# audiohacking/fp8-mps-metal

Hardware: AMD Instinct MI355X
Metric: FP8 _scaled_mm TFLOPS (M>=4) + GEMV HBM GB/s (M=1) vs roofline, 1/8 GPU (higher is better)
Workload: dtype fp8_e4m3fn (fp8 MFMA into fp32 accumulators); 1 GPU; gemm: M=512 K=4096 N=4096 e4m3fn, per-tensor scales, fp32 out, 20 rotating weight buffers; M=512, K=4096, N=4096, hip_graph=True, parallelism=single GPU, device=AMD Radeon Graphics, arch=gfx950:sramecc+:xnack-, compute_units=256, dev_kernarg=True

## Files before the change

### fp8-mps-metal_amd/csrc/diag/fp8mi_gemm_pc.hip

```cpp

#ifdef FP8MI_DIAG

#include "fp8mi_gemm_epi.h"

namespace {

template <int BM_, int BN_, int CWM_, int CWN_, int NL_, int NSTAGE_, int KS_, int ABL_ = 0>
struct PCfg {
    static constexpr int ABL = ABL_;
    static constexpr int BM = BM_, BN = BN_;
    static constexpr int kWavesM = CWM_, kWavesN = CWN_;
    static constexpr int kConsumers = CWM_ * CWN_;
    static constexpr int kLoaders = NL_;
    static constexpr int kWaves = kConsumers;
    static constexpr int kAllWaves = kConsumers + NL_;
    static constexpr int kThreads = kAllWaves * 64;
    static constexpr int kCThreads = kConsumers * 64;
    static constexpr int WM = BM_ / CWM_, WN = BN_ / CWN_;
    static constexpr int TM = WM / 16, TN = WN / 16;
    static constexpr int KS = KS_, NSTAGE = NSTAGE_, PF = NSTAGE_ - 1;
    static constexpr int kGroupsA = BM_ / 8, kGroupsB = BN_ / 8, kGroups = kGroupsA + kGroupsB;
    static constexpr int kStepBytes = (BM_ + BN_) * BK;
    static constexpr int kStageBytes = KS_ * kStepBytes;
    static constexpr int kRingBytes = NSTAGE_ * kStageBytes;
    static constexpr int JA = kGroupsA / NL_, JB = kGroupsB / NL_;
    static constexpr int kDma = KS_ * (JA + JB);
    static_assert(WM % 16 == 0 && WN % 16 == 0 && TM >= 1 && TN >= 1, "whole MFMA fragments per consumer");
    static_assert(kGroupsA % NL_ == 0 && kGroupsB % NL_ == 0 && NL_ % 2 == 0, "loaders stage whole groups; even count for the shared swizzle");
    static_assert(NSTAGE_ >= 3 && NSTAGE_ <= 6 && (NSTAGE_ - 1) * kDma <= 63, "vmcnt is a 6-bit counter");
    static_assert(kRingBytes + 16 <= 160 * 1024, "LDS is 160 KiB per CU");
};

typedef __attribute__((address_space(3))) uint8_t lds_u8;

template <int N>
FP8MI_DEVICE void wait_vm()
{
    asm volatile("s_waitcnt vmcnt(%0)" ::"n"(N) : "memory");
}

template <typename C>
FP8MI_DEVICE void wait_landed(int newer)
{
    constexpr int G = C::kDma;
    if (4 * G <= 63 && newer >= 4) wait_vm<(4 * G <= 63 ? 4 * G : 0)>();
    else if (3 * G <= 63 && newer == 3) wait_vm<(3 * G <= 63 ? 3 * G : 0)>();
    else if (2 * G <= 63 && newer == 2) wait_vm<(2 * G <= 63 ? 2 * G : 0)>();
    else if (newer == 1) wait_vm<G>();
    else wait_vm<0>();
}

template <typename C>
struct LoadPlan {
    uint32_t va0, vb0;
    uint32_t row0;
    uint32_t kpos;
    uint32_t sa, sb;
    int rows_a, rows_b;
    bool full;
};

template <typename C, bool TAIL>
FP8MI_DEVICE void issue_stage(const LoadPlan<C> &pl, __amdgpu_buffer_rsrc_t ra, __amdgpu_buffer_rsrc_t rb, lds_u8 *stage,
                              int lw, int k0, int64_t K)
{
#pragma unroll
    for (int q = 0; q < C::KS; ++q) {
#pragma unroll
        for (int j = 0; j < C::JA + C::JB; ++j) {
            const bool is_a = j < C::JA;
            const int jo = is_a ? j : j - C::JA;
            const int gs = q * C::kGroups + (is_a ? 0 : C::kGroupsA) + lw + jo * C::kLoaders;
            uint32_t vo = (is_a ? pl.va0 + jo * pl.sa : pl.vb0 + jo * pl.sb) + q * BK;
            if (!pl.full && (int)(pl.row0 + jo * C::kLoaders * 8) >= (is_a ? pl.rows_a : pl.rows_b)) vo = kOOB;
            if (TAIL && (int64_t)k0 + q * BK + pl.kpos >= K) vo = kOOB;
            lds_void *dst = (lds_void *)(stage + gs * 1024);
            if constexpr (C::ABL & 4) { asm volatile("" ::"v"(vo), "s"(dst)); continue; }
            if (is_a) __builtin_amdgcn_raw_ptr_buffer_load_lds(ra, dst, 16, (int)vo, k0, 0, 0);
            else __builtin_amdgcn_raw_ptr_buffer_load_lds(rb, dst, 16, (int)vo, k0, 0, 0);
        }
    }
}

template <typename C>
FP8MI_DEVICE void load_loop(const LoadPlan<C> &pl, __amdgpu_buffer_rsrc_t ra, __amdgpu_buffer_rsrc_t rb, lds_u8 *smem, int lw,
                            int s0, int ns, int64_t K)
{
    constexpr int kStageK = BK * C::KS;
    const int last = (int)((K + kStageK - 1) / kStageK) - 1;
    auto issue = [&](int s, int slot) {
        const int sg = s0 + s;
        if (sg >= last) issue_stage<C, true>(pl, ra, rb, smem + slot * C::kStageBytes, lw, sg * kStageK, K);
        else issue_stage<C, false>(pl, ra, rb, smem + slot * C::kStageBytes, lw, sg * kStageK, K);
    };
#pragma unroll
    for (int s = 0; s < C::PF; ++s)
        if (s < ns) issue(s, s);
    int fill = C::PF % C::NSTAGE;
    for (int t = 0; t < ns; ++t) {
        wait_landed<C>(min(C::PF - 1, ns - 1 - t));
        __builtin_amdgcn_s_barrier();
        if (t + C::PF < ns) issue(t + C::PF, fill);
        fill = (fill + 1 == C::NSTAGE) ? 0 : fill + 1;
    }
}

template <typename C>
FP8MI_DEVICE void read_frags(const lds_u8 *unit, int a_row0, int b_row0, uint32_t off1, uint32_t off2, i32x8 (&xf)[C::TM],
                             i32x8 (&wf)[C::TN])
{
    const lds_u8 *sa = unit + a_row0 * BK;
    const lds_u8 *sb = unit + C::kGroupsA * 1024 + b_row0 * BK;
    if constexpr (C::ABL & 1) {
        const int j = (int)(uintptr_t)unit + (int)off1;
#pragma unroll
        for (int t = 0; t < C::TN; ++t) wf[t] = i32x8{j, 1, j, 1, j, 1, j, 1};
#pragma unroll
        for (int t = 0; t < C::TM; ++t) xf[t] = i32x8{j, j, j, j, j, j, j, j};
        return;
    }
#pragma unroll
    for (int t = 0; t < C::TN; ++t) {
        i32x4 lo = *(const __attribute__((address_space(3))) i32x4 *)(sb + t * 16 * BK + off1);
        i32x4 hi = *(const __attribute__((address_space(3))) i32x4 *)(sb + t * 16 * BK + off2);
        wf[t] = i32x8{lo[0], lo[1], lo[2], lo[3], hi[0], hi[1], hi[2], hi[3]};
    }
#pragma unroll
    for (int t = 0; t < C::TM; ++t) {
        i32x4 lo = *(const __attribute__((address_space(3))) i32x4 *)(sa + t * 16 * BK + off1);
        i32x4 hi = *(const __attribute__((address_space(3))) i32x4 *)(sa + t * 16 * BK + off2);
        xf[t] = i32x8{lo[0], lo[1], lo[2], lo[3], hi[0], hi[1], hi[2], hi[3]};
    }
}

template <typename C, bool SCRUB>
FP8MI_DEVICE void mfma_unit(i32x8 (&xf)[C::TM], i32x8 (&wf)[C::TN], f32x4 (&acc)[C::TN][C::TM])
{
    if constexpr (SCRUB) {
#pragma unroll
        for (int t = 0; t < C::TM; ++t)
#pragma unroll
            for (int j = 0; j < 8; ++j) xf[t][j] = (int)scrub_nan4((uint32_t)xf[t][j]);
#pragma unroll
        for (int t = 0; t < C::TN; ++t)
#pragma unroll
            for (int j = 0; j < 8; ++j) wf[t][j] = (int)scrub_nan4((uint32_t)wf[t][j]);
    }
    if constexpr (C::ABL & 2) {
#pragma unroll
        for (int t = 0; t < C::TM; ++t) asm volatile("" ::"v"(xf[t]));
#pragma unroll
        for (int t = 0; t < C::TN; ++t) asm volatile("" ::"v"(wf[t]));
        return;
    }
#pragma unroll
    for (int tn = 0; tn < C::TN; ++tn)
#pragma unroll
        for (int tm = 0; tm < C::TM; ++tm)
            acc[tn][tm] = __builtin_amdgcn_mfma_scale_f32_16x16x128_f8f6f4(wf[tn], xf[tm], acc[tn][tm], 0, 0, 0, kScaleOne, 0, kScaleOne);
}

#define FP8MI_PC_FENCE() __builtin_amdgcn_sched_barrier(0)

template <typename C>
FP8MI_DEVICE void pin_acc(f32x4 (&acc)[C::TN][C::TM])
{
#pragma unroll
    for (int tn = 0; tn < C::TN; ++tn)
#pragma unroll
        for (int tm = 0; tm < C::TM; ++tm) asm volatile("" : "+v"(acc[tn][tm]));
}

template <typename C, bool SCRUB>
FP8MI_DEVICE void consume_loop(const lds_u8 *smem, int wm0, int wn0, uint32_t off1, uint32_t off2, int ns,
                               f32x4 (&acc)[C::TN][C::TM])
{
    static_assert(C::KS == 1 || C::KS == 2, "the pair loop below is written for one or two K-steps per stage");
#pragma unroll
    for (int tn = 0; tn < C::TN; ++tn)
#pragma unroll
        for (int tm = 0; tm < C::TM; ++tm) acc[tn][tm] = f32x4{0.0f, 0.0f, 0.0f, 0.0f};
    if (ns == 0) return;
    i32x8 xa[C::TM], wa[C::TN], xb[C::TM], wb[C::TN];
    const lds_u8 *cur = smem;
    int slot = 0;
    auto next_stage = [&]() {
        slot = (slot + 1 == C::NSTAGE) ? 0 : slot + 1;
        cur = smem + slot * C::kStageBytes;
        asm volatile("s_waitcnt lgkmcnt(0)" ::: "memory");
        __builtin_amdgcn_s_barrier();
    };
    __builtin_amdgcn_s_barrier();
    read_frags<C>(cur, wm0, wn0, off1, off2, xa, wa);
    if constexpr (C::KS == 2) {
        for (int s = 0; s < ns; ++s) {
            read_frags<C>(cur + C::kStepBytes, wm0, wn0, off1, off2, xb, wb);
            FP8MI_PC_FENCE();
            mfma_unit<C, SCRUB>(xa, wa, acc);
            pin_acc<C>(acc);
            FP8MI_PC_FENCE();
            if (s + 1 < ns) {
                next_stage();
                read_frags<C>(cur, wm0, wn0, off1, off2, xa, wa);
            }
            FP8MI_PC_FENCE();
            mfma_unit<C, SCRUB>(xb, wb, acc);
            pin_acc<C>(acc);
            FP8MI_PC_FENCE();
        }
    } else {
        int s = 0;
        for (; s + 1 < ns; s += 2) {
            next_stage();
            read_frags<C>(cur, wm0, wn0, off1, off2, xb, wb);
            FP8MI_PC_FENCE();
            mfma_unit<C, SCRUB>(xa, wa, acc);
            pin_acc<C>(acc);
            FP8MI_PC_FENCE();
            if (s + 2 < ns) {
                next_stage();
                read_frags<C>(cur, wm0, wn0, off1, off2, xa, wa);
            }
            FP8MI_PC_FENCE();
            mfma_unit<C, SCRUB>(xb, wb, acc);
            pin_acc<C>(acc);
            FP8MI_PC_FENCE();
        }
        if (s < ns) mfma_unit<C, SCRUB>(xa, wa, acc);
    }
}

template <int BM, int BN, int CWM, int CWN, int NL, int NSTAGE, int KS, int ABL>
__global__ __launch_bounds__((PCfg<BM, BN, CWM, CWN, NL, NSTAGE, KS, ABL>::kThreads)) void gemm_pc_kernel(MMParams p_in, int tiles_m, int tiles_n,
                                                                                                    int vec_store, int nwg)
{
    using C = PCfg<BM, BN, CWM, CWN, NL, NSTAGE, KS, ABL>;
    __shared__ __attribute__((aligned(16))) uint8_t smem[C::kRingBytes + kFlagBytes];
    if (threadIdx.x == 0) *(volatile int *)(smem + C::kRingBytes) = 0;
    const MMParams p = pin_params(p_in);
    FP8MI_PIN_S(tiles_m); FP8MI_PIN_S(tiles_n); FP8MI_PIN_S(vec_store); FP8MI_PIN_S(nwg);
    const EpiScalars es = load_epi_scalars(p);

    int tile_m, tile_n, kslice, wg;
    tile_of_block(blockIdx.x, nwg, tiles_m, tiles_n, tile_m, tile_n, kslice, wg);
    const int64_t m0 = (int64_t)tile_m * BM, n0 = (int64_t)tile_n * BN;

    const int lane = threadIdx.x & 63;
    const int wave = __builtin_amdgcn_readfirstlane(threadIdx.x >> 6);
    const bool is_loader = wave >= C::kConsumers;
    const int lw = wave - C::kConsumers;

    const int64_t rows_a = min((int64_t)BM, p.M - m0), rows_b = min((int64_t)BN, p.N - n0);
    constexpr int kStageK = BK * C::KS;
    const int ns_all = (int)((p.K + kStageK - 1) / kStageK);
    const int nsplit = p.split > 1 ? p.split : 1;
    const int ns_slice = (ns_all + nsplit - 1) / nsplit;
    const int s0 = kslice * ns_slice, ns = min(ns_slice, ns_all - s0);
    lds_u8 *ring = (lds_u8 *)smem;

    volatile int *flag = (volatile int *)(smem + C::kRingBytes);

    if (is_loader) {
        const int64_t bytes_a = (rows_a - 1) * p.lda + p.K, bytes_b = (rows_b - 1) * p.ldb + p.K;
        __amdgpu_buffer_rsrc_t ra = __builtin_amdgcn_make_buffer_rsrc((void *)(p.A + m0 * p.lda), 0,
                                                                       (int)min(bytes_a, (int64_t)0x7FFFFFFF), 0x00020000);
        __amdgpu_buffer_rsrc_t rb = __builtin_amdgcn_make_buffer_rsrc((void *)(p.B + n0 * p.ldb), 0,
                                                                       (int)min(bytes_b, (int64_t)0x7FFFFFFF), 0x00020000);
        LoadPlan<C> pl;
        const int row0 = lw * 8 + (lane >> 3);
        const int chunk = (lane & 7) ^ (((lw & 1) * 4 + (lane >> 4)) & 7);
        pl.row0 = (uint32_t)row0;
        pl.kpos = (uint32_t)(chunk * 16);
        pl.va0 = (uint32_t)(row0 * p.lda + chunk * 16);
        pl.vb0 = (uint32_t)(row0 * p.ldb + chunk * 16);
        pl.sa = (uint32_t)(C::kLoaders * 8 * p.lda);
        pl.sb = (uint32_t)(C::kLoaders * 8 * p.ldb);
        pl.rows_a = (int)rows_a;
        pl.rows_b = (int)rows_b;
        pl.full = rows_a == BM && rows_b == BN;
        for (int pass = 0; pass < 2; ++pass) {
            load_loop<C>(pl, ra, rb, ring, lw, s0, ns, p.K);
            __builtin_amdgcn_s_barrier();
            if (!p.nan_zero || pass == 1 || !*flag) break;
        }
        return;
    }

    const int wm0 = (wave % C::kWavesM) * C::WM, wn0 = (wave / C::kWavesM) * C::WN;
    const int fr = lane & 15, fg = lane >> 4;
    const uint32_t off1 = (uint32_t)(fr * BK + ((fg ^ (fr >> 1)) << 4));
    const uint32_t off2 = (uint32_t)(fr * BK + (((4 + fg) ^ (fr >> 1)) << 4));
    f32x4 acc[C::TN][C::TM];
    for (int pass = 0; pass < 2; ++pass) {
        if (pass == 0) consume_loop<C, false>(ring, wm0, wn0, off1, off2, ns, acc);
        else consume_loop<C, true>(ring, wm0, wn0, off1, off2, ns, acc);
        if (p.nan_zero && pass == 0 && acc_has_nan<C>(acc)) *flag = 1;
        asm volatile("s_waitcnt lgkmcnt(0)" ::: "memory");
        __builtin_amdgcn_s_barrier();
        if (!p.nan_zero || pass == 1 || !*flag) break;
    }

    if (nsplit > 1) {
        if (!splitk_combine<C>(p, acc, smem, wg, kslice, nsplit, tiles_m * tiles_n)) return;
    }

    const int rows_m = (int)rows_a, cols_n = (int)rows_b;
    if (rows_m == BM && cols_n == BN && vec_store) {
        if (p.out_dtype == FP8MI_F32) epilogue_staged<C, FP8MI_F32>(p, es, acc, smem, m0, n0, wave, wm0, wn0, lane);
        else if (p.out_dtype == FP8MI_BF16) epilogue_staged<C, FP8MI_BF16>(p, es, acc, smem, m0, n0, wave, wm0, wn0, lane);
        else epilogue_staged<C, FP8MI_F16>(p, es, acc, smem, m0, n0, wave, wm0, wn0, lane);
    } else if (p.out_dtype == FP8MI_F32) epilogue<C, FP8MI_F32>(p, es, acc, m0, n0, wm0, wn0, fr, fg, rows_m, cols_n, vec_store);
    else if (p.out_dtype == FP8MI_BF16) epilogue<C, FP8MI_BF16>(p, es, acc, m0, n0, wm0, wn0, fr, fg, rows_m, cols_n, vec_store);
    else epilogue<C, FP8MI_F16>(p, es, acc, m0, n0, wm0, wn0, fr, fg, rows_m, cols_n, vec_store);
}

template <int BM, int BN, int CWM, int CWN, int NL, int NSTAGE, int KS, int ABL = 0>
int launch_pc(const MMParams &p_in, hipStream_t s)
{
    using C = PCfg<BM, BN, CWM, CWN, NL, NSTAGE, KS, ABL>;
    MMParams p = p_in;
    const int64_t tm = (p.M + BM - 1) / BM, tn = (p.N + BN - 1) / BN;
    if (tm * tn > 0x7FFFFFFF) return FP8MI_E_UNSUPPORTED;
    const int rc = resolve_split(p, tm, tn, BM, BN, BK * KS);
    if (rc) return rc;
    const int esz = p.out_dtype == FP8MI_F32 ? 4 : 2;
    const int vec = (((p.ldc * esz) % 16) == 0 && (((uintptr_t)p.C) % 16) == 0) ? 1 : 0;
    const unsigned grid = (unsigned)(tm * tn * p.split);
    return fp8mi_launch(gemm_pc_kernel<BM, BN, CWM, CWN, NL, NSTAGE, KS, ABL>, dim3(grid), dim3(C::kThreads), s, p, (int)tm, (int)tn, vec, (int)grid);
}

}

int fp8mi_launch_gemm_pc(const MMParams &p, int variant, hipStream_t s)
{
    switch (variant) {
    case 15: return launch_pc<128, 64, 2, 2, 4, 3, 2>(p, s);
    case 16: return launch_pc<64, 128, 2, 2, 4, 3, 2>(p, s);
    case 17: return launch_pc<128, 128, 2, 2, 4, 4, 1>(p, s);
    case 20: return launch_pc<128, 64, 4, 2, 4, 3, 2>(p, s);
    case 21: return launch_pc<128, 128, 4, 2, 4, 4, 1>(p, s);
    case 22: return launch_pc<128, 64, 2, 2, 2, 3, 2>(p, s);
    case 24: return launch_pc<128, 64, 2, 2, 4, 6, 1>(p, s);
    case 25: return launch_pc<128, 64, 2, 2, 8, 3, 2>(p, s);
    case 26: return launch_pc<128, 64, 4, 2, 8, 3, 2>(p, s);
    case 27: return launch_pc<128, 128, 2, 2, 8, 4, 1>(p, s);
    case 28: return launch_pc<128, 64, 2, 2, 8, 6, 1>(p, s);
    case 208: return launch_pc<128, 64, 2, 2, 8, 3, 2, 3>(p, s);
    case 201: return launch_pc<128, 64, 2, 2, 4, 3, 2, 1>(p, s);
    case 202: return launch_pc<128, 64, 2, 2, 4, 3, 2, 2>(p, s);
    case 203: return launch_pc<128, 64, 2, 2, 4, 3, 2, 3>(p, s);
    case 204: return launch_pc<128, 64, 2, 2, 4, 3, 2, 4>(p, s);
    case 205: return launch_pc<128, 64, 2, 2, 4, 3, 2, 5>(p, s);
    case 206: return launch_pc<128, 64, 2, 2, 4, 3, 2, 6>(p, s);
    case 207: return launch_pc<128, 64, 2, 2, 4, 3, 2, 7>(p, s);
    default: return FP8MI_E_ENUM;
    }
}

#endif
```

### fp8-mps-metal_amd/csrc/fp8mi_common.h

```cpp
#pragma once

#include <hip/hip_runtime.h>
#include <hip/hip_ext.h>
#include <stdint.h>
#include <type_traits>

#include "../../include/fp8mi.h"

typedef float    f32x2  __attribute__((ext_vector_type(2)));
typedef float    f32x4  __attribute__((ext_vector_type(4)));
typedef float    f32x16 __attribute__((ext_vector_type(16)));
typedef int      i32x4  __attribute__((ext_vector_type(4)));
typedef int      i32x8  __attribute__((ext_vector_type(8)));
typedef uint32_t u32x2  __attribute__((ext_vector_type(2)));
typedef uint32_t u32x4  __attribute__((ext_vector_type(4)));
typedef _Float16 f16x2  __attribute__((ext_vector_type(2)));

#define FP8MI_DEVICE __device__ __forceinline__

struct MMParams {
    const uint8_t *A;
    const uint8_t *B;
    void *C;
    const float *scale_a;
    const float *scale_b;
    const void *bias;
    const float *scale_result;
    int64_t M, N, K;
    int64_t lda, ldb, ldc;
    int sa_row, sb_row;
    int out_dtype, bias_dtype;
    int transposed;
    int nan_zero;
    int debug;
    int split;
    uint8_t *ws;
    int64_t ws_bytes;
};

constexpr int kWsCounterBytes = 4096;

struct MxScales {
    const uint8_t *sx, *sw;
    int64_t ld_sx, ld_sw;
};

struct BwScales {
    const float *sa, *sb;
    int64_t sa_sr, sa_sk, sb_sr, sb_sk;
    int64_t nkb;
    int sh_a, sh_b;
};

struct QuantOut {
    uint8_t *out;
    int64_t ld_out;
    void *scales;
    int64_t s_sr, s_sk;
    int mx_flags;
    float *amax;
};

struct NqArgs {
    const void *in;
    int64_t rows, cols, ld_in;
    float eps;
    const void *weight, *bias, *mod_scale, *mod_shift;
    int64_t ld_mod, rows_per_mod;
    int param_dtype;
    const void *residual;
    int64_t ld_res;
    void *h_out;
    int64_t ld_h;
    QuantOut q;
    float *mean_out, *rstd_out;
};

#define FP8MI_PIN_S(x) asm volatile("" : "+s"(x))
FP8MI_DEVICE MMParams pin_params(const MMParams &p)
{
    MMParams q = p;
    FP8MI_PIN_S(q.A); FP8MI_PIN_S(q.B); FP8MI_PIN_S(q.C); FP8MI_PIN_S(q.scale_a); FP8MI_PIN_S(q.scale_b);
    FP8MI_PIN_S(q.bias); FP8MI_PIN_S(q.scale_result);
    FP8MI_PIN_S(q.M); FP8MI_PIN_S(q.N); FP8MI_PIN_S(q.K); FP8MI_PIN_S(q.lda); FP8MI_PIN_S(q.ldb); FP8MI_PIN_S(q.ldc);
    FP8MI_PIN_S(q.sa_row); FP8MI_PIN_S(q.sb_row); FP8MI_PIN_S(q.out_dtype); FP8MI_PIN_S(q.bias_dtype);
    FP8MI_PIN_S(q.transposed); FP8MI_PIN_S(q.nan_zero); FP8MI_PIN_S(q.split); FP8MI_PIN_S(q.ws); FP8MI_PIN_S(q.ws_bytes);
    return q;
}

#ifndef FP8MI_CSTORE
#define FP8MI_CSTORE 1
#endif
constexpr int kCStoreAux = FP8MI_CSTORE == 0 ? 0 : FP8MI_CSTORE == 1 ? 2 : FP8MI_CSTORE == 2 ? 17 : FP8MI_CSTORE == 3 ? 19 : FP8MI_CSTORE == 4 ? 16 : 18;
FP8MI_DEVICE void store_c16(u32x4 q, void *ptr)
{
#if FP8MI_CSTORE == 0
    *(u32x4 *)ptr = q;
#elif FP8MI_CSTORE == 1
    __builtin_nontemporal_store(q, (u32x4 *)ptr);
#elif FP8MI_CSTORE == 2
    asm volatile("global_store_dwordx4 %0, %1, off sc0 sc1" ::"v"(ptr), "v"(q) : "memory");
#elif FP8MI_CSTORE == 3
    asm volatile("global_store_dwordx4 %0, %1, off sc0 sc1 nt" ::"v"(ptr), "v"(q) : "memory");
#elif FP8MI_CSTORE == 4
    asm volatile("global_store_dwordx4 %0, %1, off sc1" ::"v"(ptr), "v"(q) : "memory");
#else
    asm volatile("global_store_dwordx4 %0, %1, off sc1 nt" ::"v"(ptr), "v"(q) : "memory");
#endif
}

FP8MI_DEVICE uint32_t scrub_nan4(uint32_t w)
{
    uint32_t n = ~(w | 0x80808080u);
    uint32_t m = ~((n + 0x7F7F7F7Fu) | 0x7F7F7F7Fu);
    m = m | (m - (m >> 7));
    return w & ~m;
}

FP8MI_DEVICE bool has_nan4(uint32_t w)
{
    uint32_t n = ~(w | 0x80808080u);
    return (~((n + 0x7F7F7F7Fu) | 0x7F7F7F7Fu)) != 0u;
}

FP8MI_DEVICE float decode_ref(uint32_t b)
{
    const uint32_t mag = b & 0x7Fu;
    if (mag == 0x7Fu) return 0.0f;
    const uint32_t sign = (b & 0x80u) << 24;
    uint32_t bits;
    if (mag >= 8u) bits = (mag << 20) + (120u << 23);
    else bits = __float_as_uint((float)mag * 0x1p-9f);
    return __uint_as_float(bits | sign);
}

FP8MI_DEVICE float decode_e5m2(uint32_t b) { return (float)__builtin_bit_cast(_Float16, (uint16_t)((b & 0xFFu) << 8)); }
FP8MI_DEVICE float decode_fmt(uint32_t b, int e5m2) { return e5m2 ? decode_e5m2(b) : __builtin_amdgcn_cvt_f32_fp8((int)b, 0); }

FP8MI_DEVICE float e2m1_value(uint32_t c)
{
    const uint32_t e = (c >> 1) & 3u, m = c & 1u;
    const float v = e == 0 ? 0.5f * (float)m : (float)((2u + m) << (e - 1)) * 0.5f;
    return (c & 8u) ? -v : v;
}

FP8MI_DEVICE float load_as_float(const void *p, int64_t i, int dtype)
{
    if (dtype == FP8MI_F32) return ((const float *)p)[i];
    if (dtype == FP8MI_F16) return (float)((const _Float16 *)p)[i];
    return (float)((const __bf16 *)p)[i];
}

FP8MI_DEVICE void store_from_float(void *p, int64_t i, float v, int dtype)
{
    if (dtype == FP8MI_F32) ((float *)p)[i] = v;
    else if (dtype == FP8MI_F16) ((_Float16 *)p)[i] = (_Float16)v;
    else ((__bf16 *)p)[i] = (__bf16)v;
}

FP8MI_DEVICE float epilogue_value(float sum, float sa, float sb, bool has_bias, float bias,
                                  bool has_sr, float sr, bool transposed = false)
{
    float r = transposed ? (sum * sb) * sa : (sum * sa) * sb;
    if (has_bias) r = r + bias;
    if (has_sr) r = r * sr;
    return r;
}

template <int CTRL>
FP8MI_DEVICE float dpp_add(float x)
{
    const int y = __builtin_amdgcn_update_dpp(0, __builtin_bit_cast(int, x), CTRL, 0xF, 0xF, false);
    return x + __builtin_bit_cast(float, y);
}

template <int P>
FP8MI_DEVICE float group_sum(float v)
{
    static_assert(P == 1 || P == 2 || P == 4 || P == 8 || P == 16, "a power of two inside a row of 16 lanes");
    if (P >= 2) v = dpp_add<0xB1>(v);
    if (P >= 4) v = dpp_add<0x4E>(v);
    if (P >= 8) v = dpp_add<0x141>(v);
    if (P >= 16) v = dpp_add<0x140>(v);
    return v;
}

FP8MI_DEVICE float wave_sum(float v)
{
    v = group_sum<16>(v);
    const int b = __builtin_bit_cast(int, v);
    const float r0 = __builtin_bit_cast(float, __builtin_amdgcn_readlane(b, 0)), r1 = __builtin_bit_cast(float, __builtin_amdgcn_readlane(b, 16)),
                r2 = __builtin_bit_cast(float, __builtin_amdgcn_readlane(b, 32)), r3 = __builtin_bit_cast(float, __builtin_amdgcn_readlane(b, 48));
    return (r0 + r1) + (r2 + r3);
}

bool fp8mi_next_profile_events(hipEvent_t *start, hipEvent_t *stop);

template <typename... KArgs>
int fp8mi_launch(void (*kernel)(KArgs...), dim3 grid, dim3 block, hipStream_t s, KArgs... args)
{
    void *argv[] = {(void *)&args...};
    hipEvent_t e0, e1;
    if (fp8mi_next_profile_events(&e0, &e1))
        return (int)hipExtLaunchKernel((const void *)kernel, grid, block, argv, 0, s, e0, e1, 0);
    return (int)hipLaunchKernel((const void *)kernel, grid, block, argv, 0, s);
}

int fp8mi_cu_count();

int fp8mi_launch_gemv(const MMParams &p, bool fp32_only, hipStream_t s, int fmt = 0);
int fp8mi_launch_gemv_variant(const MMParams &p, int id, hipStream_t s);
bool fp8mi_gemv_supported(const MMParams &p);
int fp8mi_launch_gemv_mx(const MMParams &p, hipStream_t s, int fmt = 0);
bool fp8mi_gemv_mx_supported(const MMParams &p);
int fp8mi_launch_gemv_mx_variant(const MMParams &p, int id, hipStream_t s);
int fp8mi_launch_gemm(const MMParams &p, int variant, hipStream_t s, int fmt = 0);
int fp8mi_choose_gemm_variant(const MMParams &p);
bool fp8mi_gemm_supported(const MMParams &p);
int fp8mi_launch_gemm256(const MMParams &p, int variant, hipStream_t s);
int fp8mi_launch_gemm256_fmt(const MMParams &p, int variant, hipStream_t s, int fmt);
bool fp8mi_gemm256_supported(const MMParams &p);
int fp8mi_launch_generic(const MMParams &p, hipStream_t s, int fmt = 0);
int fp8mi_launch_generic_mxfp8(const MMParams &p, const MxScales &sc, hipStream_t s);
int fp8mi_launch_gemm_mxfp8(const MMParams &p, const MxScales &sc, int variant, hipStream_t s);
bool fp8mi_gemm_mxfp8_supported(const MMParams &p, const MxScales &sc);
int fp8mi_choose_gemm_mxfp8_variant(const MMParams &p);
int fp8mi_launch_generic_mxfp4(const MMParams &p, const MxScales &sc, hipStream_t s);
int fp8mi_launch_gemm_mxfp4(const MMParams &p, const MxScales &sc, int variant, hipStream_t s);
bool fp8mi_gemm_mxfp4_supported(const MMParams &p, const MxScales &sc);
int fp8mi_launch_generic_blockwise(const MMParams &p, const BwScales &sc, hipStream_t s);
int fp8mi_launch_gemm_blockwise(const MMParams &p, const BwScales &sc, int variant, hipStream_t s);
bool fp8mi_gemm_blockwise_supported(const MMParams &p, const BwScales &sc);
int fp8mi_launch_skinny(const MMParams &p, hipStream_t s, int fmt = 0);
int fp8mi_launch_gemm_pc(const MMParams &p, int variant, hipStream_t s);
bool fp8mi_skinny_supported(const MMParams &p);
```

### fp8-mps-metal_amd/csrc/fp8mi_gemm.hip

```cpp

#include "fp8mi_gemm_epi.h"
#include "fp8mi_dispatch.h"

namespace {

template <int BM, int BN, int WM, int WN, int NSTAGE_, int MODE_ = 0, int ABL_ = 0, int KS_ = 1, int LD_ = 0, int MXS_ = 0, int FMT_ = 0>
struct Cfg {
    static constexpr int FW = (FMT_ >> 1) & 1, FX = FMT_ & 1;
    static constexpr bool OCP = FMT_ != 0;
    static_assert(FMT_ >= 0 && FMT_ <= 3 && (FMT_ == 0 || MXS_ == 0), "the block-scaled and blockwise forms are e4m3 / e2m1 only");

    static constexpr int KS = KS_;
    static constexpr int PFD = ABL_ & 7;
    static constexpr int PFA = (ABL_ >> 3) & 1;
    static constexpr int FLOOR = (ABL_ >> 4) & 3;
    static constexpr bool BREG = ((ABL_ >> 6) & 1) != 0;
    static constexpr bool XLOCAL = ((ABL_ >> 7) & 1) != 0;
    static constexpr int MODE = MODE_;
    static constexpr int NSTAGE = NSTAGE_;
    static constexpr int PF = NSTAGE_ - 1;
    static constexpr int kWavesM = BM / WM;
    static constexpr int kWavesN = BN / WN;
    static constexpr int kWaves = kWavesM * kWavesN;
    static constexpr int kThreads = kWaves * 64;
    static constexpr int kCThreads = kThreads;
    static constexpr int TM = WM / 16;
    static constexpr int TN = WN / 16;
    static constexpr int kGroupsA = BM / 8;
    static constexpr int kGroupsB = BN / 8;
    static constexpr int kGroups = kGroupsA + kGroupsB;
    static constexpr int kStepBytes = (BM + BN) * BK;
    static constexpr int kLoaders = LD_ == 0 ? kWaves : LD_;
    static constexpr int kGroupsPerWave = KS_ * kGroups / kLoaders;
    static constexpr bool MXS = MXS_ != 0;
    static constexpr bool FP4 = MXS_ == 2;
    static constexpr bool BW = MXS_ == 3;
    static constexpr int kScaleHalves = FP4 ? 2 : 1;
    static constexpr int kScalePiecesA = (BM + 63) / 64, kScalePieces = kScalePiecesA + (BN + 63) / 64;
    static constexpr int kScaleLoadsPerWave = MXS ? (KS_ * kScaleHalves * kScalePieces + kLoaders - 1) / kLoaders : 0;
    static constexpr int kScaleBytes = MXS ? (kScaleLoadsPerWave * kLoaders * 256 + 1023) / 1024 * 1024 : 0;
    static constexpr int kLoadsPerWave = kGroupsPerWave + kScaleLoadsPerWave;
    static constexpr int kStageBytes = KS_ * kStepBytes + kScaleBytes;
    static_assert(kGroupsA % kLoaders == 0 && kGroupsB % kLoaders == 0 && kLoaders % 2 == 0 && kLoaders <= kWaves,
                  "each loading wave stages whole groups of both operands; the shared swizzle needs an even count");
    static constexpr int kRingBytes = NSTAGE_ * kStageBytes;
    static_assert(NSTAGE_ >= 2 && NSTAGE_ <= 6 && (NSTAGE_ - 1) * kLoadsPerWave <= 63, "vmcnt is a 6-bit counter");
    static_assert(kRingBytes + 16 <= 160 * 1024, "LDS is 160 KiB per CU");
    static_assert(MODE_ >= 0 && MODE_ <= 2 && (MODE_ != 2 || KS_ == 1), "three orders of the loop body are built (the staggered one for KS = 1)");
};

template <typename C, bool SCRUB>
FP8MI_DEVICE void load_frags(const uint8_t *a_rows, const uint8_t *b_rows, int a_row0 , int b_row0 ,
                             uint32_t off1, uint32_t off2, i32x8 (&xf)[C::TM], i32x8 (&wf)[C::TN])
{
    const uint8_t *sa = a_rows + a_row0 * BK;
    const uint8_t *sB = b_rows + b_row0 * BK;
#pragma unroll
    for (int t = 0; t < C::TM; ++t) {
        i32x4 lo = *(const i32x4 *)(sa + t * 16 * BK + off1);
        i32x4 hi = *(const i32x4 *)(sa + t * 16 * BK + off2);
        xf[t] = i32x8{lo[0], lo[1], lo[2], lo[3], hi[0], hi[1], hi[2], hi[3]};
    }
#pragma unroll
    for (int t = 0; t < C::TN; ++t) {
        i32x4 lo = *(const i32x4 *)(sB + t * 16 * BK + off1);
        i32x4 hi = *(const i32x4 *)(sB + t * 16 * BK + off2);
        wf[t] = i32x8{lo[0], lo[1], lo[2], lo[3], hi[0], hi[1], hi[2], hi[3]};
    }
    if (SCRUB) {
#pragma unroll
        for (int t = 0; t < C::TM; ++t)
#pragma unroll
            for (int j = 0; j < 8; ++j) xf[t][j] = (int)scrub_nan4((uint32_t)xf[t][j]);
#pragma unroll
        for (int t = 0; t < C::TN; ++t)
#pragma unroll
            for (int j = 0; j < 8; ++j) wf[t][j] = (int)scrub_nan4((uint32_t)wf[t][j]);
    }
}

template <typename C>
FP8MI_DEVICE void mfma_all(const i32x8 (&xf)[C::TM], const i32x8 (&wf)[C::TN], f32x4 (&acc)[C::TN][C::TM])
{
#pragma unroll
    for (int tn = 0; tn < C::TN; ++tn)
#pragma unroll
        for (int tm = 0; tm < C::TM; ++tm)
            acc[tn][tm] = __builtin_amdgcn_mfma_scale_f32_16x16x128_f8f6f4(wf[tn], xf[tm], acc[tn][tm], C::FW, C::FX, 0,
                                                                            kScaleOne, 0, kScaleOne);
}

template <typename C, bool SCRUB>
FP8MI_DEVICE void compute_step(const uint8_t *stage, int a_row0, int b_row0, uint32_t off1, uint32_t off2,
                               f32x4 (&acc)[C::TN][C::TM])
{
    i32x8 xf[C::TM], wf[C::TN];
    load_frags<C, SCRUB>(stage, stage + C::kGroupsA * 1024, a_row0, b_row0, off1, off2, xf, wf);
    mfma_all<C>(xf, wf, acc);
}


template <typename C, bool = C::MXS> struct MxLane { };
template <typename C> struct MxLane<C, true> {
    uint32_t xo, wo;
    uint32_t rows_ok;
    int64_t kend;
};

template <typename C> struct StepScales { uint32_t x[(C::TM + 3) / 4], w[(C::TN + 3) / 4]; };

template <typename C>
FP8MI_DEVICE void load_scales(const uint8_t *sc, const MxLane<C, true> &ml, int64_t kstep, StepScales<C> &s, int koff = 0)
{
    const bool kin = kstep * BK + koff < ml.kend;
#pragma unroll
    for (int t = 0; t < (C::TM + 3) / 4; ++t) s.x[t] = 0u;
#pragma unroll
    for (int t = 0; t < (C::TN + 3) / 4; ++t) s.w[t] = 0u;
#pragma unroll
    for (int t = 0; t < C::TM; ++t) {
        const uint32_t b = sc[ml.xo + t * 64];
        s.x[t >> 2] |= ((kin && ((ml.rows_ok >> t) & 1u)) ? b : 0x7Fu) << (8 * (t & 3));
    }
#pragma unroll
    for (int t = 0; t < C::TN; ++t) {
        const uint32_t b = sc[ml.wo + t * 64];
        s.w[t >> 2] |= ((kin && ((ml.rows_ok >> (16 + t)) & 1u)) ? b : 0x7Fu) << (8 * (t & 3));
    }
}

FP8MI_DEVICE f32x4 mfma_mx(i32x8 w, i32x8 x, f32x4 c, uint32_t sw, int ow, uint32_t sx, int ox)
{
#define FP8MI_MX_CASE(a, b) \
    case a * 4 + b: return __builtin_amdgcn_mfma_scale_f32_16x16x128_f8f6f4(w, x, c, 0, 0, a, (int)sw, b, (int)sx);
    switch (ow * 4 + ox) {
        FP8MI_MX_CASE(0, 0) FP8MI_MX_CASE(0, 1) FP8MI_MX_CASE(0, 2) FP8MI_MX_CASE(0, 3)
        FP8MI_MX_CASE(1, 0) FP8MI_MX_CASE(1, 1) FP8MI_MX_CASE(1, 2) FP8MI_MX_CASE(1, 3)
        FP8MI_MX_CASE(2, 0) FP8MI_MX_CASE(2, 1) FP8MI_MX_CASE(2, 2) FP8MI_MX_CASE(2, 3)
        FP8MI_MX_CASE(3, 0) FP8MI_MX_CASE(3, 1) FP8MI_MX_CASE(3, 2) FP8MI_MX_CASE(3, 3)
    default: return c;
    }
#undef FP8MI_MX_CASE
}

template <typename C>
FP8MI_DEVICE void mfma_all(const i32x8 (&xf)[C::TM], const i32x8 (&wf)[C::TN], f32x4 (&acc)[C::TN][C::TM], const StepScales<C> &s)
{
#pragma unroll
    for (int tn = 0; tn < C::TN; ++tn)
#pragma unroll
        for (int tm = 0; tm < C::TM; ++tm)
            acc[tn][tm] = mfma_mx(wf[tn], xf[tm], acc[tn][tm], s.w[tn >> 2], tn & 3, s.x[tm >> 2], tm & 3);
}


FP8MI_DEVICE f32x4 mfma_mx4(i32x8 w, i32x8 x, f32x4 c, uint32_t sw, int ow, uint32_t sx, int ox)
{
#define FP8MI_MX4_CASE(a, b) \
    case a * 4 + b: return __builtin_amdgcn_mfma_scale_f32_16x16x128_f8f6f4(w, x, c, 4, 4, a, (int)sw, b, (int)sx);
    switch (ow * 4 + ox) {
        FP8MI_MX4_CASE(0, 0) FP8MI_MX4_CASE(0, 1) FP8MI_MX4_CASE(0, 2) FP8MI_MX4_CASE(0, 3)
        FP8MI_MX4_CASE(1, 0) FP8MI_MX4_CASE(1, 1) FP8MI_MX4_CASE(1, 2) FP8MI_MX4_CASE(1, 3)
        FP8MI_MX4_CASE(2, 0) FP8MI_MX4_CASE(2, 1) FP8MI_MX4_CASE(2, 2) FP8MI_MX4_CASE(2, 3)
        FP8MI_MX4_CASE(3, 0) FP8MI_MX4_CASE(3, 1) FP8MI_MX4_CASE(3, 2) FP8MI_MX4_CASE(3, 3)
    default: return c;
    }
#undef FP8MI_MX4_CASE
}

FP8MI_DEVICE i32x8 frag_hi(i32x8 f) { return __builtin_shufflevector(f, f, 4, 5, 6, 7, 4, 5, 6, 7); }

template <typename C>
FP8MI_DEVICE void mfma_step_fp4(const i32x8 (&xf)[C::TM], const i32x8 (&wf)[C::TN], f32x4 (&acc)[C::TN][C::TM], const uint8_t *sc,
                                const MxLane<C> &ml, int64_t kstep)
{
    StepScales<C> s0, s1;
    load_scales<C>(sc, ml, kstep, s0);
    load_scales<C>(sc + C::kScalePieces * 256, ml, kstep, s1, 64);
#pragma unroll
    for (int tn = 0; tn < C::TN; ++tn)
#pragma unroll
        for (int tm = 0; tm < C::TM; ++tm)
            acc[tn][tm] = mfma_mx4(wf[tn], xf[tm], acc[tn][tm], s0.w[tn >> 2], tn & 3, s0.x[tm >> 2], tm & 3);
#pragma unroll
    for (int tn = 0; tn < C::TN; ++tn)
#pragma unroll
        for (int tm = 0; tm < C::TM; ++tm)
            acc[tn][tm] = mfma_mx4(frag_hi(wf[tn]), frag_hi(xf[tm]), acc[tn][tm], s1.w[tn >> 2], tn & 3, s1.x[tm >> 2], tm & 3);
}

template <typename C>
FP8MI_DEVICE void fold_bw(f32x4 &acc, const f32x4 &pb, float sa, const f32x4 &sb)
{
#pragma unroll
    for (int j = 0; j < 4; ++j) {
        float s = sa * sb[j];
        asm("" : "+v"(s));
        float r = __builtin_fmaf(pb[j], s, acc[j]);
        asm("" : "+v"(r));
        acc[j] = r;
    }
}

template <typename C>
FP8MI_DEVICE void mfma_fold_bw(const i32x8 (&xf)[C::TM], const i32x8 (&wf)[C::TN], f32x4 (&acc)[C::TN][C::TM], const uint8_t *sc,
                               const MxLane<C> &ml)
{
    float sa[C::TM];
    f32x4 sb[C::TN];
#pragma unroll
    for (int t = 0; t < C::TM; ++t) sa[t] = *(const float *)(sc + ml.xo + t * 64);
#pragma unroll
    for (int t = 0; t < C::TN; ++t) sb[t] = *(const f32x4 *)(sc + ml.wo + t * 64);
    f32x4 prev = f32x4{0.0f, 0.0f, 0.0f, 0.0f};
#pragma unroll
    for (int i = 0; i < C::TN * C::TM; ++i) {
        const int tn = i / C::TM, tm = i % C::TM;
        const f32x4 cur = __builtin_amdgcn_mfma_scale_f32_16x16x128_f8f6f4(wf[tn], xf[tm], f32x4{0.0f, 0.0f, 0.0f, 0.0f}, 0, 0, 0,
                                                                          kScaleOne, 0, kScaleOne);
        if (i > 0) fold_bw<C>(acc[(i - 1) / C::TM][(i - 1) % C::TM], prev, sa[(i - 1) % C::TM], sb[(i - 1) / C::TM]);
        prev = cur;
    }
    constexpr int kLast = C::TN * C::TM - 1;
    fold_bw<C>(acc[kLast / C::TM][kLast % C::TM], prev, sa[kLast % C::TM], sb[kLast / C::TM]);
}

template <typename C, bool SCRUB>
FP8MI_DEVICE void compute_step(const uint8_t *stage, int q, int a_row0, int b_row0, uint32_t off1, uint32_t off2,
                               const MxLane<C> &ml, int64_t kstep, f32x4 (&acc)[C::TN][C::TM])
{
    if constexpr (C::BW) {
        i32x8 xf[C::TM], wf[C::TN];
        const uint8_t *st = stage + q * C::kStepBytes;
        load_frags<C, SCRUB>(st, st + C::kGroupsA * 1024, a_row0, b_row0, off1, off2, xf, wf);
        mfma_fold_bw<C>(xf, wf, acc, stage + C::KS * C::kStepBytes + q * C::kScalePieces * 256, ml);
    } else if constexpr (C::FP4) {
        i32x8 xf[C::TM], wf[C::TN];
        const uint8_t *st = stage + q * C::kStepBytes;
        load_frags<C, false>(st, st + C::kGroupsA * 1024, a_row0, b_row0, off1, off2, xf, wf);
        mfma_step_fp4<C>(xf, wf, acc, stage + C::KS * C::kStepBytes + q * 2 * C::kScalePieces * 256, ml, kstep);
    } else if constexpr (C::MXS) {
        i32x8 xf[C::TM], wf[C::TN];
        StepScales<C> sc;
        const uint8_t *st = stage + q * C::kStepBytes;
        load_frags<C, SCRUB>(st, st + C::kGroupsA * 1024, a_row0, b_row0, off1, off2, xf, wf);
        load_scales<C>(stage + C::KS * C::kStepBytes + q * C::kScalePieces * 256, ml, kstep, sc);
        mfma_all<C>(xf, wf, acc, sc);
    } else {
        compute_step<C, SCRUB>(stage + q * C::kStepBytes, a_row0, b_row0, off1, off2, acc);
    }
}

template <typename C, bool = C::MXS> struct ScaleStage { };
template <typename C> struct ScaleStage<C, true> {
    __amdgpu_buffer_rsrc_t rx, rw;
    uint32_t voff[C::kScaleLoadsPerWave];
    bool is_x[C::kScaleLoadsPerWave];
    uint32_t kx, kw;
    int nkb;
    int q[C::kScaleLoadsPerWave];
};

template <typename C>
struct StagePlan {
    uint32_t va0, vb0;
    uint32_t row0;
    uint32_t kpos;
    uint32_t sa, sb;
    int rows_a, rows_b;
    bool full;
    uint32_t pf_off;
    u32x4 pf_rsrc;
    int pf_waves;
    mutable u32x4 bsink;
    ScaleStage<C> sc;
};

template <typename C, bool TAIL>
FP8MI_DEVICE void issue_stage(const StagePlan<C> &pl, __amdgpu_buffer_rsrc_t ra, __amdgpu_buffer_rsrc_t rb,
                              uint8_t *stage, int wave, int k0, int64_t K)
{
    constexpr int JA = C::kGroupsA / C::kLoaders, JB = C::kGroupsB / C::kLoaders, JS = JA + JB;
    if (C::kLoaders < C::kWaves && wave >= C::kLoaders) return;
#pragma unroll
    for (int j = 0; j < C::kGroupsPerWave; ++j) {
        const int q = j / JS, jj = j % JS;
        const bool is_a = jj < JA;
        const int jo = is_a ? jj : jj - JA;
        const int gs = q * C::kGroups + (is_a ? 0 : C::kGroupsA) + wave + jo * C::kLoaders;
        uint32_t vo = (is_a ? pl.va0 + jo * pl.sa : pl.vb0 + jo * pl.sb) + q * BK;
        if (!pl.full && (int)(pl.row0 + jo * C::kLoaders * 8) >= (is_a ? pl.rows_a : pl.rows_b)) vo = kOOB;
        if (TAIL && (int64_t)k0 + q * BK + pl.kpos >= K) vo = kOOB;
        lds_void *dst = (lds_void *)(stage + gs * 1024);
        if (is_a) __builtin_amdgcn_raw_ptr_buffer_load_lds(ra, dst, 16, (int)vo, k0, 0, 0);
        else if constexpr (C::BREG) asm volatile("buffer_load_dwordx4 %0, %1, %2, %3 offen" : "+v"(pl.bsink) : "v"(vo), "s"(pl.pf_rsrc), "s"((uint32_t)k0) : "memory");
        else __builtin_amdgcn_raw_ptr_buffer_load_lds(rb, dst, 16, (int)vo, k0, 0, 0);
    }
    if constexpr (C::BW) {
        const int kb = k0 / BK;
#pragma unroll
        for (int j = 0; j < C::kScaleLoadsPerWave; ++j) {
            lds_void *dst = (lds_void *)(stage + C::KS * C::kStepBytes + (wave + j * C::kLoaders) * 256);
            const uint32_t vo = kb + pl.sc.q[j] < pl.sc.nkb ? pl.sc.voff[j] + (uint32_t)kb * (pl.sc.is_x[j] ? pl.sc.kx : pl.sc.kw) : kOOB;
            __builtin_amdgcn_raw_ptr_buffer_load_lds(pl.sc.is_x[j] ? pl.sc.rx : pl.sc.rw, dst, 4, (int)vo, 0, 0, 0);
        }
    } else if constexpr (C::MXS) {
#pragma unroll
        for (int j = 0; j < C::kScaleLoadsPerWave; ++j) {
            lds_void *dst = (lds_void *)(stage + C::KS * C::kStepBytes + (wave + j * C::kLoaders) * 256);
            __builtin_amdgcn_raw_ptr_buffer_load_lds(pl.sc.is_x[j] ? pl.sc.rx : pl.sc.rw, dst, 4, (int)pl.sc.voff[j], C::FP4 ? k0 / 16 : k0 / 32, 0, 0);
        }
    }
}

#ifdef FP8MI_STAMP
#define STAMP(var)                                                                 \
    do {                                                                           \
        __builtin_amdgcn_sched_barrier(0);                                         \
        unsigned long long t_;                                                     \
        asm volatile("s_memtime %0\n\ts_waitcnt lgkmcnt(0)" : "=s"(t_)::"memory"); \
        __builtin_amdgcn_sched_barrier(0);                                         \
        var = t_;                                                                  \
    } while (0)
__device__ unsigned long long g_stamp[256 * 32];
#else
#define STAMP(var) do { } while (0)
#endif

template <int N>
FP8MI_DEVICE void wait_loads_and_lds()
{
    asm volatile("s_waitcnt vmcnt(%0) lgkmcnt(0)" ::"n"(N) : "memory");
}

template <typename C>
FP8MI_DEVICE void wait_stage(int newer_stages)
{
    constexpr int G = C::kLoadsPerWave;
    if (5 * G <= 63 && newer_stages >= 5) wait_loads_and_lds<(5 * G <= 63 ? 5 * G : 0)>();
    else if (4 * G <= 63 && newer_stages == 4) wait_loads_and_lds<(4 * G <= 63 ? 4 * G : 0)>();
    else if (3 * G <= 63 && newer_stages == 3) wait_loads_and_lds<(3 * G <= 63 ? 3 * G : 0)>();
    else if (2 * G <= 63 && newer_stages == 2) wait_loads_and_lds<(2 * G <= 63 ? 2 * G : 0)>();
    else if (newer_stages == 1) wait_loads_and_lds<G>();
    else wait_loads_and_lds<0>();
}

template <typename C>
FP8MI_DEVICE void issue_any(const StagePlan<C> &pl, __amdgpu_buffer_rsrc_t ra, __amdgpu_buffer_rsrc_t rb,
                            uint8_t *stage, int wave, int step, int nk, bool ktail, int64_t K)
{
    if (ktail && step == nk - 1) issue_stage<C, true>(pl, ra, rb, stage, wave, step * (BK * C::KS), K);
    else issue_stage<C, false>(pl, ra, rb, stage, wave, step * (BK * C::KS), K);
}

FP8MI_DEVICE void prefetch_stage(uint32_t &sink, uint32_t voff, u32x4 rsrc, uint32_t koff)
{
    asm volatile("buffer_load_dword %0, %1, %2, %3 offen" : "+v"(sink) : "v"(voff), "s"(rsrc), "s"(koff) : "memory");
}

template <typename C, bool SCRUB>
FP8MI_DEVICE void run_tile(const MMParams &p, uint8_t *smem, const StagePlan<C> &pl, __amdgpu_buffer_rsrc_t ra,
                           __amdgpu_buffer_rsrc_t rb, int wave, int wm0, int wn0, uint32_t off1, uint32_t off2,
                           int ks0, int nk, int rot, const MxLane<C> &ml, f32x4 (&acc)[C::TN][C::TM])
{
#pragma unroll
    for (int tn = 0; tn < C::TN; ++tn)
#pragma unroll
        for (int tm = 0; tm < C::TM; ++tm) acc[tn][tm] = f32x4{0.0f, 0.0f, 0.0f, 0.0f};

    const int64_t K = p.K;
    const int nk_all = (int)((K + BK * C::KS - 1) / (BK * C::KS));
    const bool ktail = (K % (BK * C::KS)) != 0;
    if (nk == 0) return;
    unsigned long long p0_ = 0, p1_ = 0, p2_ = 0; (void)p0_; (void)p1_; (void)p2_;
    STAMP(p0_);

    int ks = rot;
    auto next_ks = [&]() { const int r = ks; ks = (ks + 1 == nk) ? 0 : ks + 1; return ks0 + r; };
    uint32_t sink = 0;
    auto prefetch = [&](int stage) {
        if (C::PFD > 0 && wave < pl.pf_waves + C::PFA) prefetch_stage(sink, pl.pf_off, pl.pf_rsrc, (uint32_t)((ks0 + min(stage, nk - 1)) * (BK * C::KS)));
    };

#pragma unroll
    for (int s = 0; s < C::PF; ++s)
        if (s < nk) issue_any<C>(pl, ra, rb, smem + s * C::kStageBytes, wave, next_ks(), nk_all, ktail, K);
#pragma unroll
    for (int s = 0; s < C::PFD; ++s) prefetch(C::PF + s);

    STAMP(p1_);
    int slot = 0;
    int fill = C::PF % C::NSTAGE;
    unsigned long long c_wait = 0, c_bar = 0, c_issue = 0, c_comp = 0, s0 = 0, s1 = 0, s2 = 0, s3 = 0, s4 = 0;
    (void)c_wait; (void)c_bar; (void)c_issue; (void)c_comp; (void)s0; (void)s1; (void)s2; (void)s3; (void)s4;
    for (int t = 0; t < nk; ++t) {
        const int64_t kst = (int64_t)(ks0 + (rot + t < nk ? rot + t : rot + t - nk)) * C::KS;
        STAMP(s0);
        wait_stage<C>(min(C::PF - 1, nk - 1 - t));
        STAMP(s1);
        __builtin_amdgcn_s_barrier();
        STAMP(s2);
        if constexpr (C::MODE == 1) {
            i32x8 xf[C::TM], wf[C::TN];
            const uint8_t *st = smem + slot * C::kStageBytes;
            if constexpr (C::FLOOR == 0) load_frags<C, SCRUB>(st, st + C::kGroupsA * 1024, wm0, wn0, off1, off2, xf, wf);
            __builtin_amdgcn_sched_barrier(0);
            if (t + C::PF < nk) {
                issue_any<C>(pl, ra, rb, smem + fill * C::kStageBytes, wave, next_ks(), nk_all, ktail, K);
                prefetch(t + C::PF + C::PFD);
            }
            STAMP(s3);
            if constexpr (C::FLOOR == 0 && C::BW) {
                mfma_fold_bw<C>(xf, wf, acc, st + C::KS * C::kStepBytes, ml);
#pragma unroll
                for (int q = 1; q < C::KS; ++q) compute_step<C, SCRUB>(st, q, wm0, wn0, off1, off2, ml, kst + q, acc);
            } else if constexpr (C::FLOOR == 0 && C::FP4) {
                mfma_step_fp4<C>(xf, wf, acc, st + C::KS * C::kStepBytes, ml, kst);
#pragma unroll
                for (int q = 1; q < C::KS; ++q) compute_step<C, SCRUB>(st, q, wm0, wn0, off1, off2, ml, kst + q, acc);
            } else if constexpr (C::FLOOR == 0 && C::MXS) {
                StepScales<C> sc;
                load_scales<C>(st + C::KS * C::kStepBytes, ml, kst, sc);
                mfma_all<C>(xf, wf, acc, sc);
#pragma unroll
                for (int q = 1; q < C::KS; ++q) compute_step<C, SCRUB>(st, q, wm0, wn0, off1, off2, ml, kst + q, acc);
            } else if constexpr (C::FLOOR == 0) {
                mfma_all<C>(xf, wf, acc);
#pragma unroll
                for (int q = 1; q < C::KS; ++q)
                    compute_step<C, SCRUB>(st + q * C::kStepBytes, wm0, wn0, off1, off2, acc);
            }
        } else {
            if (t + C::PF < nk) {
                issue_any<C>(pl, ra, rb, smem + fill * C::kStageBytes, wave, next_ks(), nk_all, ktail, K);
                prefetch(t + C::PF + C::PFD);
            }
            STAMP(s3);
            if constexpr (C::FLOOR == 0 && C::MXS) {
#pragma unroll
                for (int q = 0; q < C::KS; ++q) compute_step<C, SCRUB>(smem + slot * C::kStageBytes, q, wm0, wn0, off1, off2, ml, kst + q, acc);
            } else if constexpr (C::FLOOR == 0) {
#pragma unroll
                for (int q = 0; q < C::KS; ++q)
                    compute_step<C, SCRUB>(smem + slot * C::kStageBytes + q * C::kStepBytes, wm0, wn0, off1, off2, acc);
            }
        }
        STAMP(s4);
        c_wait += s1 - s0; c_bar += s2 - s1; c_issue += s3 - s2; c_comp += s4 - s3;
#ifdef FP8MI_STAMP
        if (t == 5 && (threadIdx.x & 63) == 0 && blockIdx.x < 256 && (wave == 0 || wave == C::kWaves / 2)) {
            unsigned long long *o = g_stamp + blockIdx.x * 32 + 16 + (wave ? 5 : 0);
            o[0] = s0; o[1] = s1; o[2] = s2; o[3] = s3; o[4] = s4;
        }
#endif
        slot = (slot + 1 == C::NSTAGE) ? 0 : slot + 1;
        fill = (fill + 1 == C::NSTAGE) ? 0 : fill + 1;
    }
#ifdef FP8MI_STAMP
    if ((threadIdx.x & 63) == 0 && blockIdx.x < 256 && (wave == 0 || wave == C::kWaves / 2)) {
        unsigned long long *o = g_stamp + blockIdx.x * 32 + (wave ? 8 : 0);
        o[0] = c_wait; o[1] = c_bar; o[2] = c_issue; o[3] = c_comp; o[4] = nk;
    }
#endif
    if (C::PFD > 0) asm volatile("" ::"v"(sink));
#ifdef FP8MI_STAMP
    STAMP(p2_);
    if ((threadIdx.x & 63) == 0 && blockIdx.x < 256 && wave == 0) {
        unsigned long long *o = g_stamp + blockIdx.x * 32 + 26;
        o[0] = p0_; o[1] = p1_; o[2] = p2_;
    }
#endif
}

template <typename C, bool SCRUB>
FP8MI_DEVICE void run_tile_staggered(const MMParams &p, uint8_t *smem, const StagePlan<C> &pl, __amdgpu_buffer_rsrc_t ra,
                                     __amdgpu_buffer_rsrc_t rb, int wave, int wm0, int wn0, uint32_t off1, uint32_t off2,
                                     int ks0, int nk, int rot, const MxLane<C> &ml, f32x4 (&acc)[C::TN][C::TM])
{
    static_assert(C::KS == 1, "one K-step per ring stage");
    static_assert(!C::FP4 && !C::BW, "the MXFP4 and blockwise instances are built on the MODE 0 / 1 loops");
#pragma unroll
    for (int tn = 0; tn < C::TN; ++tn)
#pragma unroll
        for (int tm = 0; tm < C::TM; ++tm) acc[tn][tm] = f32x4{0.0f, 0.0f, 0.0f, 0.0f};
    const int64_t K = p.K;
    const int nk_all = (int)((K + BK - 1) / BK);
    const bool ktail = (K % BK) != 0;
    if (nk == 0) return;
    int ks = rot;
    auto next_ks = [&]() { const int r = ks; ks = (ks + 1 == nk) ? 0 : ks + 1; return ks0 + r; };
#pragma unroll
    for (int s = 0; s < C::PF; ++s)
        if (s < nk) issue_any<C>(pl, ra, rb, smem + s * C::kStageBytes, wave, next_ks(), nk_all, ktail, K);
    int slot = 0, fill = C::PF % C::NSTAGE;
    auto advance = [&]() {
        slot = (slot + 1 == C::NSTAGE) ? 0 : slot + 1;
        fill = (fill + 1 == C::NSTAGE) ? 0 : fill + 1;
    };
    i32x8 xf[C::TM], wf[C::TN];
    StepScales<C> sc;
#define FP8MI_READ_STEP(st, t)                                                                                                   \
    do {                                                                                                                         \
        load_frags<C, SCRUB>(st, st + C::kGroupsA * 1024, wm0, wn0, off1, off2, xf, wf);                                          \
        if constexpr (C::MXS) load_scales<C>(st + C::kStepBytes, ml, (int64_t)(ks0 + (rot + t < nk ? rot + t : rot + t - nk)), sc); \
    } while (0)
#define FP8MI_MULTIPLY()                                        \
    do {                                                        \
        if constexpr (C::MXS) mfma_all<C>(xf, wf, acc, sc);     \
        else mfma_all<C>(xf, wf, acc);                          \
    } while (0)
    if (wave < C::kWaves / 2) {
        for (int t = 0; t < nk; ++t) {
            wait_stage<C>(min(C::PF - 1, nk - 1 - t));
            __builtin_amdgcn_s_barrier();
            const uint8_t *st = smem + slot * C::kStageBytes;
            FP8MI_READ_STEP(st, t);
            __builtin_amdgcn_sched_barrier(0);
            if (t + C::PF < nk) issue_any<C>(pl, ra, rb, smem + fill * C::kStageBytes, wave, next_ks(), nk_all, ktail, K);
            FP8MI_MULTIPLY();
            advance();
        }
    } else {
        for (int t = 0; t < nk; ++t) {
            wait_stage<C>(min(C::PF - 1, nk - 1 - t));
            __builtin_amdgcn_s_barrier();
            if (t > 0) {
                FP8MI_MULTIPLY();
#pragma unroll
                for (int tn = 0; tn < C::TN; ++tn)
#pragma unroll
                    for (int tm = 0; tm < C::TM; ++tm) asm volatile("" : "+v"(acc[tn][tm]));
            }
            asm volatile("" ::: "memory");
            __builtin_amdgcn_sched_barrier(0);
            if (t + C::PF < nk) issue_any<C>(pl, ra, rb, smem + fill * C::kStageBytes, wave, next_ks(), nk_all, ktail, K);
            const uint8_t *st = smem + slot * C::kStageBytes;
            FP8MI_READ_STEP(st, t);
            advance();
        }
        FP8MI_MULTIPLY();
    }
#undef FP8MI_READ_STEP
#undef FP8MI_MULTIPLY
}

template <typename C, bool SCRUB>
FP8MI_DEVICE void run_tile_any(const MMParams &p, uint8_t *smem, const StagePlan<C> &pl, __amdgpu_buffer_rsrc_t ra,
                               __amdgpu_buffer_rsrc_t rb, int wave, int wm0, int wn0, uint32_t off1, uint32_t off2,
                               int ks0, int nk, int rot, const MxLane<C> &ml, f32x4 (&acc)[C::TN][C::TM])
{
    if constexpr (C::MODE == 2) run_tile_staggered<C, SCRUB>(p, smem, pl, ra, rb, wave, wm0, wn0, off1, off2, ks0, nk, rot, ml, acc);
    else run_tile<C, SCRUB>(p, smem, pl, ra, rb, wave, wm0, wn0, off1, off2, ks0, nk, rot, ml, acc);
}

using MxArgs = MxScales;
struct MxParams {
    MMParams mm;
    MxArgs s;
};

template <typename C, typename S>
FP8MI_DEVICE void gemm_tile(const MMParams &p, const S &mx, const EpiScalars &es, uint8_t *smem, int tiles_m, int tiles_n,
                            int vec_store, int nwg)
{
    constexpr int BM = C::kWavesM * (C::TM * 16), BN = C::kWavesN * (C::TN * 16), WM = C::TM * 16, WN = C::TN * 16;
    if (!C::FP4 && !C::OCP && threadIdx.x == 0) *(volatile int *)(smem + C::kRingBytes) = 0;

    unsigned long long k0_ = 0, k1_ = 0, k2_ = 0; (void)k0_; (void)k1_; (void)k2_;
    STAMP(k0_);
#ifdef FP8MI_STAMP
    const unsigned long long r0_ = __builtin_amdgcn_s_memrealtime();
#endif
    int tile_m, tile_n, kslice, wg;
    tile_of_block(blockIdx.x, nwg, tiles_m, tiles_n, tile_m, tile_n, kslice, wg);
    if constexpr (C::XLOCAL) {
        const int q = nwg >> 3, r = nwg & 7, xcd = blockIdx.x & 7;
        const int wg_all = (xcd < r ? xcd * (q + 1) : r * (q + 1) + (xcd - r) * q) + ((int)blockIdx.x >> 3);
        const int split = max(p.split, 1);
        wg = wg_all / split;
        kslice = wg_all - wg * split;
        tile_m = wg % tiles_m;
        tile_n = wg / tiles_m;
    }
    const int n_tiles = tiles_m * tiles_n;
    const int64_t m0 = (int64_t)tile_m * BM, n0 = (int64_t)tile_n * BN;

    const int lane = threadIdx.x & 63;
    const int wave = __builtin_amdgcn_readfirstlane(threadIdx.x >> 6);
    const int wm0 = (wave % C::kWavesM) * WM;
    const int wn0 = (wave / C::kWavesM) * WN;

    const int64_t rows_a = min((int64_t)BM, p.M - m0), rows_b = min((int64_t)BN, p.N - n0);
    const int64_t bytes_a = (rows_a - 1) * p.lda + p.K, bytes_b = (rows_b - 1) * p.ldb + p.K;
    __amdgpu_buffer_rsrc_t ra = __builtin_amdgcn_make_buffer_rsrc((void *)(p.A + m0 * p.lda), 0,
                                                                   (int)min(bytes_a, (int64_t)0x7FFFFFFF), 0x00020000);
    __amdgpu_buffer_rsrc_t rb = __builtin_amdgcn_make_buffer_rsrc((void *)(p.B + n0 * p.ldb), 0,
                                                                   (int)min(bytes_b, (int64_t)0x7FFFFFFF), 0x00020000);

    StagePlan<C> pl;
    {
        const int row0 = wave * 8 + (lane >> 3);
        const int chunk = (lane & 7) ^ (((wave & 1) * 4 + (lane >> 4)) & 7);
        pl.row0 = (uint32_t)row0;
        pl.kpos = (uint32_t)(chunk * 16);
        pl.va0 = (uint32_t)(row0 * p.lda + chunk * 16);
        pl.vb0 = (uint32_t)(row0 * p.ldb + chunk * 16);
        pl.sa = (uint32_t)(C::kLoaders * 8 * p.lda);
        pl.sb = (uint32_t)(C::kLoaders * 8 * p.ldb);
        pl.rows_a = (int)rows_a;
        pl.rows_b = (int)rows_b;
        pl.full = rows_a == BM && rows_b == BN;
        pl.pf_off = kOOB;
        pl.pf_waves = 0;
        pl.bsink = u32x4{0u, 0u, 0u, 0u};
        if constexpr (C::BREG) {
            static_assert(C::PFD == 0, "BREG borrows the prefetch descriptor");
            const uint64_t pbr = (uint64_t)(p.B + n0 * p.ldb);
            pl.pf_rsrc = u32x4{(uint32_t)__builtin_amdgcn_readfirstlane((int)(uint32_t)pbr),
                               (uint32_t)__builtin_amdgcn_readfirstlane((int)((uint32_t)(pbr >> 32) & 0xFFFFu)),
                               (uint32_t)__builtin_amdgcn_readfirstlane((int)min(bytes_b, (int64_t)0x7FFFFFFF)), 0x00020000u};
            for (int o = (int)threadIdx.x * 16; o < C::kRingBytes; o += C::kThreads * 16) *(u32x4 *)(smem + o) = u32x4{0u, 0u, 0u, 0u};
            __syncthreads();
        }
        if (C::PFD > 0) {
            constexpr int kLines = BN * C::KS / 4;
            static_assert(C::PFD == 0 || kLines <= 64, "one prefetch instruction per stage");
            const int gm = min(4, tiles_m - (tile_m & ~3)), nshare = gm >= 4 ? 4 : (gm >= 2 ? 2 : 1);
            pl.pf_waves = nshare == 1 ? 0 : 4 / nshare;
            const int quarter = (tile_m % nshare) * (4 / nshare) + wave;
            const int li = (quarter & 3) * kLines + lane, prow = li / C::KS, pk = li % C::KS;
            if (lane < kLines && prow < (int)rows_b && (p.K % (BK * C::KS)) == 0) pl.pf_off = (uint32_t)(prow * p.ldb + pk * BK);
            const uint64_t pb = (uint64_t)(p.B + n0 * p.ldb);
            pl.pf_rsrc = u32x4{(uint32_t)__builtin_amdgcn_readfirstlane((int)(uint32_t)pb),
                               (uint32_t)__builtin_amdgcn_readfirstlane((int)((uint32_t)(pb >> 32) & 0xFFFFu)),
                               (uint32_t)__builtin_amdgcn_readfirstlane((int)min(bytes_b, (int64_t)0x7FFFFFFF)), 0x00020000u};
            if (C::PFA && wave == pl.pf_waves) {
                constexpr int kLinesA = BM * C::KS / 8;
                static_assert(!C::PFA || kLinesA <= 64, "one prefetch instruction per stage");
                const int lia = (tile_n & 7) * kLinesA + lane, arow = lia / C::KS, ak = lia % C::KS;
                pl.pf_off = (lane < kLinesA && arow < (int)rows_a && (p.K % (BK * C::KS)) == 0) ? (uint32_t)(arow * p.lda + ak * BK) : kOOB;
                const uint64_t pa = (uint64_t)(p.A + m0 * p.lda);
                pl.pf_rsrc = u32x4{(uint32_t)__builtin_amdgcn_readfirstlane((int)(uint32_t)pa),
                                   (uint32_t)__builtin_amdgcn_readfirstlane((int)((uint32_t)(pa >> 32) & 0xFFFFu)),
                                   (uint32_t)__builtin_amdgcn_readfirstlane((int)min(bytes_a, (int64_t)0x7FFFFFFF)), 0x00020000u};
            }
        }
    }

    const int fr = lane & 15, fg = lane >> 4;
    const uint32_t off1 = (uint32_t)(fr * BK + ((fg ^ (fr >> 1)) << 4));
    const uint32_t off2 = (uint32_t)(fr * BK + (((4 + fg) ^ (fr >> 1)) << 4));

    MxLane<C> ml;
    if constexpr (C::BW) {
        const int64_t bx0 = m0 >> mx.sh_a, bw0 = n0 >> mx.sh_b;
        const int64_t nbx = ((m0 + rows_a - 1) >> mx.sh_a) - bx0 + 1, nbw = ((n0 + rows_b - 1) >> mx.sh_b) - bw0 + 1;
        const int64_t ext_x = ((nbx - 1) * mx.sa_sr + (mx.nkb - 1) * mx.sa_sk + 1) * 4, ext_w = ((nbw - 1) * mx.sb_sr + (mx.nkb - 1) * mx.sb_sk + 1) * 4;
        pl.sc.rx = __builtin_amdgcn_make_buffer_rsrc((void *)(mx.sa + bx0 * mx.sa_sr), 0, (int)min(ext_x, (int64_t)0x7FFFFFFF), 0x00020000);
        pl.sc.rw = __builtin_amdgcn_make_buffer_rsrc((void *)(mx.sb + bw0 * mx.sb_sr), 0, (int)min(ext_w, (int64_t)0x7FFFFFFF), 0x00020000);
        pl.sc.kx = (uint32_t)(mx.sa_sk * 4);
        pl.sc.kw = (uint32_t)(mx.sb_sk * 4);
        pl.sc.nkb = (int)mx.nkb;
#pragma unroll
        for (int j = 0; j < C::kScaleLoadsPerWave; ++j) {
            const int idx = wave + j * C::kLoaders, q = idx / C::kScalePieces, part = idx - q * C::kScalePieces;
            const bool is_x = part < C::kScalePiecesA;
            const int row = (is_x ? part : part - C::kScalePiecesA) * 64 + lane;
            const bool ok = idx < C::KS * C::kScalePieces && row < (is_x ? rows_a : rows_b);
            const int64_t rb = is_x ? ((m0 + row) >> mx.sh_a) - bx0 : ((n0 + row) >> mx.sh_b) - bw0;
            pl.sc.voff[j] = ok ? (uint32_t)(rb * (is_x ? mx.sa_sr : mx.sb_sr) * 4 + q * (is_x ? pl.sc.kx : pl.sc.kw)) : kOOB;
            pl.sc.is_x[j] = is_x;
            pl.sc.q[j] = q;
        }
        ml.xo = (uint32_t)((wm0 + fr) * 4);
        ml.wo = (uint32_t)(C::kScalePiecesA * 256 + (wn0 + fg * 4) * 4);
        ml.rows_ok = 0;
        ml.kend = 0;
    } else if constexpr (C::MXS) {
        pl.sc.rx = __builtin_amdgcn_make_buffer_rsrc((void *)(mx.sx + m0 * mx.ld_sx), 0, (int)min(rows_a * mx.ld_sx, (int64_t)0x7FFFFFFF), 0x00020000);
        pl.sc.rw = __builtin_amdgcn_make_buffer_rsrc((void *)(mx.sw + n0 * mx.ld_sw), 0, (int)min(rows_b * mx.ld_sw, (int64_t)0x7FFFFFFF), 0x00020000);
#pragma unroll
        for (int j = 0; j < C::kScaleLoadsPerWave; ++j) {
            const int idx = wave + j * C::kLoaders, q = idx / C::kScalePieces, part = idx - q * C::kScalePieces;
            const bool is_x = part < C::kScalePiecesA;
            const int row = (is_x ? part : part - C::kScalePiecesA) * 64 + lane;
            const bool ok = idx < C::KS * C::kScaleHalves * C::kScalePieces && row < (is_x ? rows_a : rows_b);
            pl.sc.voff[j] = ok ? (uint32_t)(row * (is_x ? mx.ld_sx : mx.ld_sw) + q * 4) : kOOB;
            pl.sc.is_x[j] = is_x;
        }
        ml.xo = (uint32_t)((wm0 + fr) * 4 + fg);
        ml.wo = (uint32_t)(C::kScalePiecesA * 256 + (wn0 + fr) * 4 + fg);
        uint32_t ok = 0;
#pragma unroll
        for (int t = 0; t < C::TM; ++t) ok |= (wm0 + t * 16 + fr < rows_a) ? 1u << t : 0u;
#pragma unroll
        for (int t = 0; t < C::TN; ++t) ok |= (wn0 + t * 16 + fr < rows_b) ? 1u << (16 + t) : 0u;
        ml.rows_ok = ok;
        ml.kend = p.K - (C::FP4 ? 16 : 32) * fg;
    }

    const int nk_all = (int)((p.K + BK * C::KS - 1) / (BK * C::KS));
    const int nsplit = p.split > 1 ? p.split : 1;
    const int nk_slice = (nk_all + nsplit - 1) / nsplit;
    const int ks0 = kslice * nk_slice, nk = min(nk_slice, nk_all - ks0);
    const int rot = 0;

    f32x4 acc[C::TN][C::TM];
    if constexpr (C::FLOOR == 2) {
#pragma unroll
        for (int tn = 0; tn < C::TN; ++tn)
#pragma unroll
            for (int tm = 0; tm < C::TM; ++tm) acc[tn][tm] = f32x4{0.0f, 0.0f, 0.0f, 0.0f};
    } else
    run_tile_any<C, false>(p, smem, pl, ra, rb, wave, wm0, wn0, off1, off2, ks0, nk, rot, ml, acc);

    if constexpr (C::FP4 || C::OCP) {
        asm volatile("s_waitcnt lgkmcnt(0)" ::: "memory");
        __builtin_amdgcn_s_barrier();
    } else {
        volatile int *flag = (volatile int *)(smem + C::kRingBytes);
        if (p.nan_zero && acc_has_nan<C>(acc)) *flag = 1;
        asm volatile("s_waitcnt lgkmcnt(0)" ::: "memory");
        __builtin_amdgcn_s_barrier();
        if (p.nan_zero && *flag) {
            run_tile_any<C, true>(p, smem, pl, ra, rb, wave, wm0, wn0, off1, off2, ks0, nk, rot, ml, acc);
            asm volatile("s_waitcnt lgkmcnt(0)" ::: "memory");
            __builtin_amdgcn_s_barrier();
        }
    }

    if (nsplit > 1) {
#ifdef FP8MI_DIAG
        if (p.debug & 1) {
            if ((wave % C::kWavesM) * 2 / C::kWavesM != (kslice & 1)) return;
        } else
#endif
        if (!splitk_combine<C>(p, acc, smem, wg, kslice, nsplit, n_tiles)) return;
    }

    STAMP(k1_);
    const int rows_m = (int)rows_a, cols_n = (int)rows_b;
    if (rows_m == BM && cols_n == BN && vec_store) {
        if (p.out_dtype == FP8MI_F32) epilogue_staged<C, FP8MI_F32>(p, es, acc, smem, m0, n0, wave, wm0, wn0, lane);
        else if (p.out_dtype == FP8MI_BF16) epilogue_staged<C, FP8MI_BF16>(p, es, acc, smem, m0, n0, wave, wm0, wn0, lane);
        else epilogue_staged<C, FP8MI_F16>(p, es, acc, smem, m0, n0, wave, wm0, wn0, lane);
    } else if (p.out_dtype == FP8MI_F32) epilogue<C, FP8MI_F32>(p, es, acc, m0, n0, wm0, wn0, fr, fg, rows_m, cols_n, vec_store);
    else if (p.out_dtype == FP8MI_BF16) epilogue<C, FP8MI_BF16>(p, es, acc, m0, n0, wm0, wn0, fr, fg, rows_m, cols_n, vec_store);
    else epilogue<C, FP8MI_F16>(p, es, acc, m0, n0, wm0, wn0, fr, fg, rows_m, cols_n, vec_store);
#ifdef FP8MI_STAMP
    asm volatile("s_waitcnt vmcnt(0)" ::: "memory");
    STAMP(k2_);
    if (threadIdx.x == 0 && blockIdx.x < 256) {
        g_stamp[blockIdx.x * 32 + 5] = k1_ - k0_;
        g_stamp[blockIdx.x * 32 + 6] = k2_ - k1_;
        g_stamp[blockIdx.x * 32 + 7] = __builtin_amdgcn_s_memrealtime() - r0_;
        g_stamp[blockIdx.x * 32 + 29] = k0_;
        g_stamp[blockIdx.x * 32 + 30] = k1_;
    }
#endif
}

template <int BM, int BN, int WM, int WN, int NSTAGE, int PP, int ABL, int KS, int LD>
__global__ __launch_bounds__((Cfg<BM, BN, WM, WN, NSTAGE, PP, ABL, KS, LD>::kThreads)) void gemm_kernel(MMParams p_in, int tiles_m, int tiles_n, int vec_store, int nwg)
{
    using C = Cfg<BM, BN, WM, WN, NSTAGE, PP, ABL, KS, LD>;
    const MMParams p = pin_params(p_in);
    FP8MI_PIN_S(tiles_m); FP8MI_PIN_S(tiles_n); FP8MI_PIN_S(vec_store); FP8MI_PIN_S(nwg);
    if constexpr (C::FLOOR == 3) {
        if (p.M < 0) *(volatile int *)p.C = tiles_m + tiles_n + vec_store + nwg;
        return;
    }
    const EpiScalars es = load_epi_scalars(p);
    __shared__ __attribute__((aligned(16))) uint8_t smem[C::kRingBytes + kFlagBytes];
    if (threadIdx.x == 0) *(volatile int *)(smem + C::kRingBytes) = 0;

    unsigned long long k0_ = 0, k1_ = 0, k2_ = 0; (void)k0_; (void)k1_; (void)k2_;
    STAMP(k0_);
#ifdef FP8MI_STAMP
    const unsigned long long r0_ = __builtin_amdgcn_s_memrealtime();
#endif
    int tile_m, tile_n, kslice, wg;
    tile_of_block(blockIdx.x, nwg, tiles_m, tiles_n, tile_m, tile_n, kslice, wg);
    if constexpr (C::XLOCAL) {
        const int q = nwg >> 3, r = nwg & 7, xcd = blockIdx.x & 7;
        const int wg_all = (xcd < r ? xcd * (q + 1) : r * (q + 1) + (xcd - r) * q) + ((int)blockIdx.x >> 3);
        const int split = max(p.split, 1);
        wg = wg_all / split;
        kslice = wg_all - wg * split;
        tile_m = wg % tiles_m;
        tile_n = wg / tiles_m;
    }
    const int n_tiles = tiles_m * tiles_n;
    const int64_t m0 = (int64_t)tile_m * BM, n0 = (int64_t)tile_n * BN;

    const int lane = threadIdx.x & 63;
    const int wave = __builtin_amdgcn_readfirstlane(threadIdx.x >> 6);
    const int wm0 = (wave % C::kWavesM) * WM;
    const int wn0 = (wave / C::kWavesM) * WN;

    const int64_t rows_a = min((int64_t)BM, p.M - m0), rows_b = min((int64_t)BN, p.N - n0);
    const int64_t bytes_a = (rows_a - 1) * p.lda + p.K, bytes_b = (rows_b - 1) * p.ldb + p.K;
    __amdgpu_buffer_rsrc_t ra = __builtin_amdgcn_make_buffer_rsrc((void *)(p.A + m0 * p.lda), 0,
                                                                   (int)min(bytes_a, (int64_t)0x7FFFFFFF), 0x00020000);
    __amdgpu_buffer_rsrc_t rb = __builtin_amdgcn_make_buffer_rsrc((void *)(p.B + n0 * p.ldb), 0,
                                                                   (int)min(bytes_b, (int64_t)0x7FFFFFFF), 0x00020000);

    StagePlan<C> pl;
    {
        const int row0 = wave * 8 + (lane >> 3);
        const int chunk = (lane & 7) ^ (((wave & 1) * 4 + (lane >> 4)) & 7);
        pl.row0 = (uint32_t)row0;
        pl.kpos = (uint32_t)(chunk * 16);
        pl.va0 = (uint32_t)(row0 * p.lda + chunk * 16);
        pl.vb0 = (uint32_t)(row0 * p.ldb + chunk * 16);
        pl.sa = (uint32_t)(C::kLoaders * 8 * p.lda);
        pl.sb = (uint32_t)(C::kLoaders * 8 * p.ldb);
        pl.rows_a = (int)rows_a;
        pl.rows_b = (int)rows_b;
        pl.full = rows_a == BM && rows_b == BN;
        pl.pf_off = kOOB;
        pl.pf_waves = 0;
        pl.bsink = u32x4{0u, 0u, 0u, 0u};
        if constexpr (C::BREG) {
            static_assert(C::PFD == 0, "BREG borrows the prefetch descriptor");
            const uint64_t pbr = (uint64_t)(p.B + n0 * p.ldb);
            pl.pf_rsrc = u32x4{(uint32_t)__builtin_amdgcn_readfirstlane((int)(uint32_t)pbr),
                               (uint32_t)__builtin_amdgcn_readfirstlane((int)((uint32_t)(pbr >> 32) & 0xFFFFu)),
                               (uint32_t)__builtin_amdgcn_readfirstlane((int)min(bytes_b, (int64_t)0x7FFFFFFF)), 0x00020000u};
            for (int o = (int)threadIdx.x * 16; o < C::kRingBytes; o += C::kThreads * 16) *(u32x4 *)(smem + o) = u32x4{0u, 0u, 0u, 0u};
            __syncthreads();
        }
        if (C::PFD > 0) {
            constexpr int kLines = BN * C::KS / 4;
            static_assert(C::PFD == 0 || kLines <= 64, "one prefetch instruction per stage");
            const int gm = min(4, tiles_m - (tile_m & ~3)), nshare = gm >= 4 ? 4 : (gm >= 2 ? 2 : 1);
            pl.pf_waves = nshare == 1 ? 0 : 4 / nshare;
            const int quarter = (tile_m % nshare) * (4 / nshare) + wave;
            const int li = (quarter & 3) * kLines + lane, prow = li / C::KS, pk = li % C::KS;
            if (lane < kLines && prow < (int)rows_b && (p.K % (BK * C::KS)) == 0) pl.pf_off = (uint32_t)(prow * p.ldb + pk * BK);
            const uint64_t pb = (uint64_t)(p.B + n0 * p.ldb);
            pl.pf_rsrc = u32x4{(uint32_t)__builtin_amdgcn_readfirstlane((int)(uint32_t)pb),
                               (uint32_t)__builtin_amdgcn_readfirstlane((int)((uint32_t)(pb >> 32) & 0xFFFFu)),
                               (uint32_t)__builtin_amdgcn_readfirstlane((int)min(bytes_b, (int64_t)0x7FFFFFFF)), 0x00020000u};
            if (C::PFA && wave == pl.pf_waves) {
                constexpr int kLinesA = BM * C::KS / 8;
                static_assert(!C::PFA || kLinesA <= 64, "one prefetch instruction per stage");
                const int lia = (tile_n & 7) * kLinesA + lane, arow = lia / C::KS, ak = lia % C::KS;
                pl.pf_off = (lane < kLinesA && arow < (int)rows_a && (p.K % (BK * C::KS)) == 0) ? (uint32_t)(arow * p.lda + ak * BK) : kOOB;
                const uint64_t pa = (uint64_t)(p.A + m0 * p.lda);
                pl.pf_rsrc = u32x4{(uint32_t)__builtin_amdgcn_readfirstlane((int)(uint32_t)pa),
                                   (uint32_t)__builtin_amdgcn_readfirstlane((int)((uint32_t)(pa >> 32) & 0xFFFFu)),
                                   (uint32_t)__builtin_amdgcn_readfirstlane((int)min(bytes_a, (int64_t)0x7FFFFFFF)), 0x00020000u};
            }
        }
    }

    const int fr = lane & 15, fg = lane >> 4;
    const uint32_t off1 = (uint32_t)(fr * BK + ((fg ^ (fr >> 1)) << 4));
    const uint32_t off2 = (uint32_t)(fr * BK + (((4 + fg) ^ (fr >> 1)) << 4));

    const int nk_all = (int)((p.K + BK * C::KS - 1) / (BK * C::KS));
    const int nsplit = p.split > 1 ? p.split : 1;
    const int nk_slice = (nk_all + nsplit - 1) / nsplit;
    const int ks0 = kslice * nk_slice, nk = min(nk_slice, nk_all - ks0);
    const int rot = 0;

    f32x4 acc[C::TN][C::TM];
    if constexpr (C::FLOOR == 2) {
#pragma unroll
        for (int tn = 0; tn < C::TN; ++tn)
#pragma unroll
            for (int tm = 0; tm < C::TM; ++tm) acc[tn][tm] = f32x4{0.0f, 0.0f, 0.0f, 0.0f};
    } else
    run_tile_any<C, false>(p, smem, pl, ra, rb, wave, wm0, wn0, off1, off2, ks0, nk, rot, MxLane<C>{}, acc);

    volatile int *flag = (volatile int *)(smem + C::kRingBytes);
    if (p.nan_zero && acc_has_nan<C>(acc)) *flag = 1;
    asm volatile("s_waitcnt lgkmcnt(0)" ::: "memory");
    __builtin_amdgcn_s_barrier();
    if (p.nan_zero && *flag) {
        run_tile_any<C, true>(p, smem, pl, ra, rb, wave, wm0, wn0, off1, off2, ks0, nk, rot, MxLane<C>{}, acc);
        asm volatile("s_waitcnt lgkmcnt(0)" ::: "memory");
        __builtin_amdgcn_s_barrier();
    }

    if (nsplit > 1) {
#ifdef FP8MI_DIAG
        if (p.debug & 1) {
            if ((wave % C::kWavesM) * 2 / C::kWavesM != (kslice & 1)) return;
        } else
#endif
        if (!splitk_combine<C>(p, acc, smem, wg, kslice, nsplit, n_tiles)) return;
    }

    STAMP(k1_);
    const int rows_m = (int)rows_a, cols_n = (int)rows_b;
    if (rows_m == BM && cols_n == BN && vec_store) {
        if (p.out_dtype == FP8MI_F32) epilogue_staged<C, FP8MI_F32>(p, es, acc, smem, m0, n0, wave, wm0, wn0, lane);
        else if (p.out_dtype == FP8MI_BF16) epilogue_staged<C, FP8MI_BF16>(p, es, acc, smem, m0, n0, wave, wm0, wn0, lane);
        else epilogue_staged<C, FP8MI_F16>(p, es, acc, smem, m0, n0, wave, wm0, wn0, lane);
    } else if (p.out_dtype == FP8MI_F32) epilogue<C, FP8MI_F32>(p, es, acc, m0, n0, wm0, wn0, fr, fg, rows_m, cols_n, vec_store);
    else if (p.out_dtype == FP8MI_BF16) epilogue<C, FP8MI_BF16>(p, es, acc, m0, n0, wm0, wn0, fr, fg, rows_m, cols_n, vec_store);
    else epilogue<C, FP8MI_F16>(p, es, acc, m0, n0, wm0, wn0, fr, fg, rows_m, cols_n, vec_store);
#ifdef FP8MI_STAMP
    asm volatile("s_waitcnt vmcnt(0)" ::: "memory");
    STAMP(k2_);
    if (threadIdx.x == 0 && blockIdx.x < 256) {
        g_stamp[blockIdx.x * 32 + 5] = k1_ - k0_;
        g_stamp[blockIdx.x * 32 + 6] = k2_ - k1_;
        g_stamp[blockIdx.x * 32 + 7] = __builtin_amdgcn_s_memrealtime() - r0_;
        g_stamp[blockIdx.x * 32 + 29] = k0_;
        g_stamp[blockIdx.x * 32 + 30] = k1_;
    }
#endif
}

template <int BM, int BN, int WM, int WN, int NSTAGE, int PP, int ABL, int KS, int LD>
__global__ __launch_bounds__((Cfg<BM, BN, WM, WN, NSTAGE, PP, ABL, KS, LD, 1>::kThreads)) void gemm_mxfp8_kernel(MxParams px, int tiles_m, int tiles_n, int vec_store, int nwg)
{
    using C = Cfg<BM, BN, WM, WN, NSTAGE, PP, ABL, KS, LD, 1>;
    static_assert(C::FLOOR == 0 && !C::BREG && !C::XLOCAL, "the block-scaled form is built from product configurations only");
    const MMParams p = pin_params(px.mm);
    MxArgs mx = px.s;
    FP8MI_PIN_S(mx.sx); FP8MI_PIN_S(mx.sw); FP8MI_PIN_S(mx.ld_sx); FP8MI_PIN_S(mx.ld_sw);
    FP8MI_PIN_S(tiles_m); FP8MI_PIN_S(tiles_n); FP8MI_PIN_S(vec_store); FP8MI_PIN_S(nwg);
    EpiScalars es;
    es.sa0 = 1.0f;
    es.sb0 = 1.0f;
    es.sr = p.scale_result ? p.scale_result[0] : 1.0f;
    __shared__ __attribute__((aligned(16))) uint8_t smem[C::kRingBytes + kFlagBytes];
    gemm_tile<C>(p, mx, es, smem, tiles_m, tiles_n, vec_store, nwg);
}

template <int BM, int BN, int WM, int WN, int NSTAGE, int PP, int ABL, int KS, int LD>
__global__ __launch_bounds__((Cfg<BM, BN, WM, WN, NSTAGE, PP, ABL, KS, LD, 2>::kThreads)) void gemm_mxfp4_kernel(MxParams px, int tiles_m, int tiles_n, int vec_store, int nwg)
{
    using C = Cfg<BM, BN, WM, WN, NSTAGE, PP, ABL, KS, LD, 2>;
    static_assert(C::FLOOR == 0 && !C::BREG && !C::XLOCAL, "the block-scaled form is built from product configurations only");
    const MMParams p = pin_params(px.mm);
    MxArgs mx = px.s;
    FP8MI_PIN_S(mx.sx); FP8MI_PIN_S(mx.sw); FP8MI_PIN_S(mx.ld_sx); FP8MI_PIN_S(mx.ld_sw);
    FP8MI_PIN_S(tiles_m); FP8MI_PIN_S(tiles_n); FP8MI_PIN_S(vec_store); FP8MI_PIN_S(nwg);
    EpiScalars es;
    es.sa0 = 1.0f;
    es.sb0 = 1.0f;
    es.sr = p.scale_result ? p.scale_result[0] : 1.0f;
    __shared__ __attribute__((aligned(16))) uint8_t smem[C::kRingBytes + kFlagBytes];
    gemm_tile<C>(p, mx, es, smem, tiles_m, tiles_n, vec_store, nwg);
}

struct BwParams {
    MMParams mm;
    BwScales s;
};

template <int BM, int BN, int WM, int WN, int NSTAGE, int PP, int ABL, int KS, int LD>
__global__ __launch_bounds__((Cfg<BM, BN, WM, WN, NSTAGE, PP, ABL, KS, LD, 3>::kThreads)) void gemm_blockwise_kernel(BwParams px, int tiles_m, int tiles_n, int vec_store, int nwg)
{
    using C = Cfg<BM, BN, WM, WN, NSTAGE, PP, ABL, KS, LD, 3>;
    static_assert(C::FLOOR == 0 && !C::BREG && !C::XLOCAL, "the blockwise form is built from product configurations only");
    static_assert(128 % BM == 0 && 128 % BN == 0, "a tile lies inside one 128-row scale block");
    const MMParams p = pin_params(px.mm);
    BwScales bs = px.s;
    FP8MI_PIN_S(bs.sa); FP8MI_PIN_S(bs.sb); FP8MI_PIN_S(bs.sa_sr); FP8MI_PIN_S(bs.sa_sk); FP8MI_PIN_S(bs.sb_sr); FP8MI_PIN_S(bs.sb_sk);
    FP8MI_PIN_S(bs.nkb); FP8MI_PIN_S(bs.sh_a); FP8MI_PIN_S(bs.sh_b);
    FP8MI_PIN_S(tiles_m); FP8MI_PIN_S(tiles_n); FP8MI_PIN_S(vec_store); FP8MI_PIN_S(nwg);
    EpiScalars es;
    es.sa0 = 1.0f;
    es.sb0 = 1.0f;
    es.sr = p.scale_result ? p.scale_result[0] : 1.0f;
    __shared__ __attribute__((aligned(16))) uint8_t smem[C::kRingBytes + kFlagBytes];
    gemm_tile<C>(p, bs, es, smem, tiles_m, tiles_n, vec_store, nwg);
}

#ifndef FP8MI_FLOOR_PROBE
struct NoScales { };

template <int FMT, int BM, int BN, int WM, int WN, int NSTAGE, int PP, int ABL, int KS, int LD>
__global__ __launch_bounds__((Cfg<BM, BN, WM, WN, NSTAGE, PP, ABL, KS, LD, 0, FMT>::kThreads)) void gemm_fmt_kernel(MMParams p_in, int tiles_m, int tiles_n, int vec_store, int nwg)
{
    using C = Cfg<BM, BN, WM, WN, NSTAGE, PP, ABL, KS, LD, 0, FMT>;
    static_assert(C::OCP && C::FLOOR == 0 && !C::BREG && !C::XLOCAL, "the e5m2 forms are built from product configurations only");
    const MMParams p = pin_params(p_in);
    FP8MI_PIN_S(tiles_m); FP8MI_PIN_S(tiles_n); FP8MI_PIN_S(vec_store); FP8MI_PIN_S(nwg);
    const EpiScalars es = load_epi_scalars(p);
    __shared__ __attribute__((aligned(16))) uint8_t smem[C::kRingBytes + kFlagBytes];
    gemm_tile<C>(p, NoScales{}, es, smem, tiles_m, tiles_n, vec_store, nwg);
}

#endif

inline MMParams &mm_of(MMParams &p) { return p; }
template <class P> MMParams &mm_of(P &px) { return px.mm; }

template <class C, int BM, int BN, class Params>
int launch_ring(void (*kernel)(Params, int, int, int, int), Params px, hipStream_t s)
{
    MMParams &p = mm_of(px);
    const int64_t tm = (p.M + BM - 1) / BM, tn = (p.N + BN - 1) / BN;
    if (tm * tn > 0x7FFFFFFF) return FP8MI_E_UNSUPPORTED;
    const int rc = resolve_split(p, tm, tn, BM, BN, BK * C::KS);
    if (rc) return rc;
    const int esz = p.out_dtype == FP8MI_F32 ? 4 : 2;
    const int vec = (((p.ldc * esz) % 16) == 0 && (((uintptr_t)p.C) % 16) == 0) ? 1 : 0;
    const unsigned grid = (unsigned)(tm * tn * p.split);
    return fp8mi_launch(kernel, dim3(grid), dim3(C::kThreads), s, px, (int)tm, (int)tn, vec, (int)grid);
}

template <int BM, int BN, int... R>
struct Tile { };

template <int BM, int BN, int WM, int WN, int NSTAGE, int PP = 0, int ABL = 0, int KS = 1, int LD = 0>
int launch(const MMParams &p, hipStream_t s)
{
    return launch_ring<Cfg<BM, BN, WM, WN, NSTAGE, PP, ABL, KS, LD>, BM, BN>(gemm_kernel<BM, BN, WM, WN, NSTAGE, PP, ABL, KS, LD>, p, s);
}

template <int BM, int BN, int... R>
int launch(Tile<BM, BN, R...>, const MMParams &p, hipStream_t s)
{
    return launch<BM, BN, R...>(p, s);
}

#ifndef FP8MI_FLOOR_PROBE
template <int FMT, int BM, int BN, int... R>
int launch_fmt(Tile<BM, BN, R...>, const MMParams &p, hipStream_t s)
{
    return launch_ring<Cfg<BM, BN, R..., 0, FMT>, BM, BN>(gemm_fmt_kernel<FMT, BM, BN, R...>, p, s);
}
#endif

template <int MXS, int BM, int BN, int... R>
int launch_mx(Tile<BM, BN, R...>, const MMParams &p, const MxScales &sc, hipStream_t s)
{
    MxParams px;
    px.mm = p;
    px.s = sc;
    if constexpr (MXS == 2) return launch_ring<Cfg<BM, BN, R..., 2>, BM, BN>(gemm_mxfp4_kernel<BM, BN, R...>, px, s);
    else return launch_ring<Cfg<BM, BN, R..., 1>, BM, BN>(gemm_mxfp8_kernel<BM, BN, R...>, px, s);
}

template <int BM, int BN, int... R>
int launch_bw(Tile<BM, BN, R...>, const MMParams &p, const BwScales &sc, hipStream_t s)
{
    BwParams px;
    px.mm = p;
    px.s = sc;
    return launch_ring<Cfg<BM, BN, R..., 3>, BM, BN>(gemm_blockwise_kernel<BM, BN, R...>, px, s);
}

template <class F>
int with_product_tile(int id, int otherwise, F &&f)
{
    switch (id) {
    case FP8MI_KERNEL_GEMM_128: return f(Tile<128, 128, 64, 32, 2, 0, 0, 1, 4>{});
    case FP8MI_KERNEL_GEMM_128x64: return f(Tile<128, 64, 32, 32, 3, 1, 1, 2, 4>{});
    case FP8MI_KERNEL_GEMM_64x128: return f(Tile<64, 128, 32, 32, 3, 1, 0, 2, 4>{});
    case FP8MI_KERNEL_GEMM_64x64: return f(Tile<64, 64, 16, 32, 4, 1, 0, 2, 4>{});
    case FP8MI_KERNEL_GEMM_32x64: return f(Tile<32, 64, 16, 32, 4, 1, 0, 2, 4>{});
    case FP8MI_KERNEL_GEMM_32x32: return f(Tile<32, 32, 16, 32, 4, 1, 0, 2, 2>{});
    case FP8MI_KERNEL_GEMM_128D: return f(Tile<128, 128, 64, 32, 4, 1, 0, 1, 4>{});
    default: return otherwise;
    }
}

using Tile256 = Tile<256, 256, 128, 64, 2, 2, 0, 1, 4>;

#ifndef FP8MI_FLOOR_PROBE
template <int FMT>
int launch_gemm_fmt(const MMParams &p, int variant, hipStream_t s)
{
    switch (variant) {
    case FP8MI_KERNEL_GEMM_256: return launch_fmt<FMT>(Tile256{}, p, s);
    case FP8MI_KERNEL_GEMM_256W: return fp8mi_launch_gemm256_fmt(p, 0, s, FMT);
    case FP8MI_KERNEL_GEMM_256x128W: return fp8mi_launch_gemm256_fmt(p, 1000, s, FMT);
    default: return with_product_tile(variant, FP8MI_E_ENUM, [&](auto t) { return launch_fmt<FMT>(t, p, s); });
    }
}
#endif


}

#ifdef FP8MI_STAMP
extern "C" int fp8mi_debug_read_stamps(unsigned long long *out, int n)
{
    return (int)hipMemcpyFromSymbol(out, HIP_SYMBOL(g_stamp), sizeof(unsigned long long) * n);
}
#endif

bool fp8mi_gemm_supported(const MMParams &p)
{
    return p.M >= 1 && p.N >= 1 && p.K >= 0 && (p.K % 16) == 0 && (p.lda % 16) == 0 && (p.ldb % 16) == 0 &&
           (((uintptr_t)p.A) & 15u) == 0 && (((uintptr_t)p.B) & 15u) == 0 && p.lda < (1 << 22) && p.ldb < (1 << 22);
}

int fp8mi_choose_gemm_variant(const MMParams &p)
{
    const double cus = (double)fp8mi_cu_count();
    int best = FP8MI_KERNEL_GEMM_128x64;
    double best_us = 1e300;
    for (const fp8mi_dispatch::TileCost &t : fp8mi_dispatch::kTileCosts) {
        const double us = fp8mi_dispatch::predict_us(p, t.id, cus);
        if (us >= 0.0 && us < best_us) { best_us = us; best = t.id; }
    }
    return best;
}

int fp8mi_launch_gemm(const MMParams &p, int variant, hipStream_t s, int fmt)
{
    if (variant == FP8MI_KERNEL_AUTO) variant = fp8mi_choose_gemm_variant(p);
#ifndef FP8MI_FLOOR_PROBE
    if (fmt == 1) return launch_gemm_fmt<1>(p, variant, s);
    if (fmt == 2) return launch_gemm_fmt<2>(p, variant, s);
    if (fmt == 3) return launch_gemm_fmt<3>(p, variant, s);
#endif
    if (fmt != 0) return FP8MI_E_UNSUPPORTED;
    switch (variant) {
    case FP8MI_KERNEL_GEMM_256: return launch(Tile256{}, p, s);
    case FP8MI_KERNEL_GEMM_256W: return fp8mi_launch_gemm256(p, 0, s);
    case FP8MI_KERNEL_GEMM_256x128W: return fp8mi_launch_gemm256(p, 1000, s);
#ifdef FP8MI_FLOOR_PROBE
    case 901: return launch<128, 64, 32, 32, 3, 1, 1 | (1 << 4), 2, 4>(p, s);
    case 902: return launch<128, 64, 32, 32, 3, 1, 1 | (2 << 4), 2, 4>(p, s);
    case 903: return launch<128, 64, 32, 32, 3, 1, 1 | (3 << 4), 2, 4>(p, s);
    case 911: return launch<128, 128, 64, 32, 4, 1, 0 | (1 << 4), 1, 4>(p, s);
    case 912: return launch<128, 128, 64, 32, 4, 1, 0 | (2 << 4), 1, 4>(p, s);
    case 913: return launch<128, 128, 64, 32, 4, 1, 0 | (3 << 4), 1, 4>(p, s);
#endif
#ifdef FP8MI_DIAG
    case 30: return launch<256, 256, 128, 64, 2, 1, 0, 1, 4>(p, s);
    case 31: return launch<128, 128, 64, 32, 2, 1, 0, 1, 4>(p, s);
    case 32: return launch<128, 64, 32, 32, 3, 0, 0, 2, 4>(p, s);
    case 33: return launch<256, 256, 128, 64, 2, 1>(p, s);
    case 34: return launch<256, 256, 128, 64, 2, 0, 0, 1, 4>(p, s);
    case 35: return launch<256, 256, 128, 64, 2, 2>(p, s);
    case 36: return launch<128, 128, 64, 32, 2, 2, 0, 1, 4>(p, s);
    case 37: return launch<128, 128, 64, 32, 2, 2>(p, s);
    case 38: return launch<128, 64, 32, 32, 3, 1, 0, 2, 4>(p, s);
    case 39: return launch<128, 64, 32, 32, 3, 1, 2, 2, 4>(p, s);
    case 120: return launch<128, 128, 64, 32, 2, 0, 1, 1, 4>(p, s);
    case 121: return launch<128, 128, 64, 32, 2, 0, 2, 1, 4>(p, s);
    case 122: return launch<128, 128, 64, 32, 2, 0, 4, 1, 4>(p, s);
    case 130: return launch<128, 128, 64, 32, 2, 0, 0, 1, 4>(p, s);
    case 131: return launch<128, 128, 64, 32, 4, 1, 0, 1, 4>(p, s);
    case 132: return launch<128, 128, 64, 32, 2, 1, 0, 2, 4>(p, s);
    case 133: return launch<128, 128, 64, 32, 3, 1, 0, 1, 4>(p, s);
    case 134: return launch<128, 128, 64, 32, 4, 1, 1, 1, 4>(p, s);
    case 135: return launch<128, 128, 64, 32, 3, 1, 1, 1, 4>(p, s);
    case 136: return launch<128, 128, 64, 32, 4, 0, 0, 1, 4>(p, s);
    case 140: return launch<128, 64, 32, 32, 3, 1, 9, 2, 4>(p, s);
    case 141: return launch<128, 64, 32, 32, 3, 1, 10, 2, 4>(p, s);
    case 150: return launch<64, 64, 32, 32, 3, 1, 0, 2, 4>(p, s);
    case 151: return launch<64, 64, 32, 32, 4, 1, 0, 2, 4>(p, s);
    case 152: return launch<64, 64, 16, 32, 4, 1, 0, 2, 4>(p, s);
    case 153: return launch<32, 128, 16, 32, 3, 1, 0, 2, 4>(p, s);
    case 154: return launch<32, 64, 16, 32, 4, 1, 0, 2, 4>(p, s);
    case 155: return launch<16, 128, 16, 32, 4, 1, 0, 2, 2>(p, s);
    case 137: return launch<64, 64, 16, 32, 4, 1, 64, 2, 4>(p, s);
    case 138: return launch<32, 64, 16, 32, 4, 1, 64, 2, 4>(p, s);
    case 144: return launch<64, 64, 16, 32, 4, 1, 128, 2, 4>(p, s);
    case 139: return launch<64, 64, 16, 32, 4, 1, 16, 2, 4>(p, s);
    case 142: return launch<64, 64, 16, 32, 4, 1, 32, 2, 4>(p, s);
    case 143: return launch<64, 64, 16, 32, 4, 1, 48, 2, 4>(p, s);
    case 156: return launch<64, 64, 16, 32, 3, 1, 0, 2, 4>(p, s);
    case 157: return launch<64, 64, 16, 32, 2, 1, 0, 2, 4>(p, s);
    case 126: return launch<64, 16, 16, 16, 4, 1, 0, 2, 2>(p, s);
    case 127: return launch<64, 16, 16, 16, 6, 1, 0, 2, 2>(p, s);
    case 128: return launch<32, 16, 16, 16, 6, 1, 0, 2, 2>(p, s);
    case 158: return launch<64, 32, 16, 32, 4, 1, 0, 2, 4>(p, s);
    case 159: return launch<32, 32, 16, 32, 4, 1, 0, 2, 2>(p, s);
    case 7: return launch<128, 64, 64, 32, 6>(p, s);
    case 8: return launch<128, 128, 64, 64, 4>(p, s);
    case 9: return launch<256, 128, 64, 64, 3, 0, 0, 1, 4>(p, s);
    case 10: return launch<128, 64, 32, 32, 6>(p, s);
    case 11: return launch<256, 256, 128, 64, 2>(p, s);
    case 12: return launch<128, 64, 32, 32, 3, 0, 0, 2>(p, s);
    case 13: return launch<128, 128, 64, 32, 2>(p, s);
#endif
    default: return with_product_tile(variant, FP8MI_E_ENUM, [&](auto t) { return launch(t, p, s); });
    }
}

bool fp8mi_gemm_mxfp8_supported(const MMParams &p, const MxScales &sc)
{
    return fp8mi_gemm_supported(p) && p.K > 0 && (p.K % 32) == 0 && (sc.ld_sx % 4) == 0 && (sc.ld_sw % 4) == 0 &&
           (((uintptr_t)sc.sx) & 3u) == 0 && (((uintptr_t)sc.sw) & 3u) == 0;
}

int fp8mi_choose_gemm_mxfp8_variant(const MMParams &p)
{
    const double cus = (double)fp8mi_cu_count();
    int best = FP8MI_KERNEL_GEMM_128x64;
    double best_us = 1e300;
    for (const fp8mi_dispatch::TileCost &t : fp8mi_dispatch::kTileCosts) {
        if (t.id == FP8MI_KERNEL_GEMM_256W || t.id == FP8MI_KERNEL_GEMM_256x128W) continue;
        MMParams q = p;
        if (q.M == 1) q.M = 2;
        const double us = fp8mi_dispatch::predict_us(q, t.id, cus);
        if (us >= 0.0 && us < best_us) { best_us = us; best = t.id; }
    }
    return best;
}

int fp8mi_launch_gemm_mxfp8(const MMParams &p, const MxScales &sc, int variant, hipStream_t s)
{
    if (variant == FP8MI_KERNEL_AUTO) variant = fp8mi_choose_gemm_mxfp8_variant(p);
    return with_product_tile(variant, FP8MI_E_UNSUPPORTED, [&](auto t) { return launch_mx<1>(t, p, sc, s); });
}

bool fp8mi_gemm_mxfp4_supported(const MMParams &p, const MxScales &sc)
{
    return fp8mi_gemm_supported(p) && p.K > 0 && (sc.ld_sx % 4) == 0 && (sc.ld_sw % 4) == 0 && (((uintptr_t)sc.sx) & 3u) == 0 &&
           (((uintptr_t)sc.sw) & 3u) == 0;
}

int fp8mi_launch_gemm_mxfp4(const MMParams &p, const MxScales &sc, int variant, hipStream_t s)
{
    if (variant == FP8MI_KERNEL_AUTO) variant = fp8mi_choose_gemm_mxfp8_variant(p);
    return with_product_tile(variant, FP8MI_E_UNSUPPORTED, [&](auto t) { return launch_mx<2>(t, p, sc, s); });
}

static int64_t bw_extent_bytes(int64_t rows, int sh, int64_t sr, int64_t sk, int64_t nkb)
{
    return ((((rows - 1) >> sh)) * sr + (nkb - 1) * sk + 1) * 4;
}

bool fp8mi_gemm_blockwise_supported(const MMParams &p, const BwScales &sc)
{
    if (!fp8mi_gemm_supported(p) || p.K <= 0 || (((uintptr_t)sc.sa) & 3u) != 0 || (((uintptr_t)sc.sb) & 3u) != 0) return false;
    constexpr int64_t kMaxStride = 0x1FFFFFFF;
    if (sc.sa_sr > kMaxStride || sc.sa_sk > kMaxStride || sc.sb_sr > kMaxStride || sc.sb_sk > kMaxStride) return false;
    return bw_extent_bytes(p.M, sc.sh_a, sc.sa_sr, sc.sa_sk, sc.nkb) < 0x7FFFFFFF && bw_extent_bytes(p.N, sc.sh_b, sc.sb_sr, sc.sb_sk, sc.nkb) < 0x7FFFFFFF;
}

int fp8mi_launch_gemm_blockwise(const MMParams &p, const BwScales &sc, int variant, hipStream_t s)
{
    if (variant == FP8MI_KERNEL_AUTO) variant = fp8mi_choose_gemm_mxfp8_variant(p);
    return with_product_tile(variant, FP8MI_E_UNSUPPORTED, [&](auto t) { return launch_bw(t, p, sc, s); });
}
```

### fp8-mps-metal_amd/csrc/fp8mi_gemm_epi.h

```cpp
#pragma once

#include "fp8mi_common.h"

namespace {

constexpr int BK = 128;
constexpr uint32_t kOOB = 0x80000000u;
constexpr int kScaleOne = 0x7F7F7F7F;
static_assert(kWsCounterBytes == FP8MI_WS_COUNTER_BYTES, "include/fp8mi.h and the kernels agree on the counter block");

typedef __attribute__((address_space(3))) void lds_void;

struct EpiScalars {
    float sa0, sb0, sr;
};

FP8MI_DEVICE EpiScalars load_epi_scalars(const MMParams &p)
{
    EpiScalars e;
    e.sa0 = p.scale_a[0];
    e.sb0 = p.scale_b[0];
    e.sr = p.scale_result ? p.scale_result[0] : 1.0f;
    return e;
}

template <typename C, int OUT>
FP8MI_DEVICE void epilogue(const MMParams &p, const EpiScalars &es, const f32x4 (&acc)[C::TN][C::TM], int64_t m0, int64_t n0, int wm0,
                           int wn0, int fr, int fg, int rows_m, int cols_n, int vec_store)
{
    const bool has_bias = p.bias != nullptr;
    const float sr = es.sr;
    const bool has_sr = p.scale_result != nullptr;
    float sbv[C::TN][4], bv[C::TN][4];
    const float sb0 = es.sb0;
#pragma unroll
    for (int tn = 0; tn < C::TN; ++tn)
#pragma unroll
        for (int j = 0; j < 4; ++j) {
            const int nl = min(wn0 + tn * 16 + fg * 4 + j, cols_n - 1);
            sbv[tn][j] = p.sb_row ? p.scale_b[n0 + nl] : sb0;
            bv[tn][j] = (has_bias && !p.transposed) ? load_as_float(p.bias, n0 + nl, p.bias_dtype) : 0.0f;
        }
    const float sa0 = es.sa0;
    constexpr int kEsz = OUT == FP8MI_F32 ? 4 : 2;
#pragma unroll
    for (int tm = 0; tm < C::TM; ++tm) {
        const int ml = wm0 + tm * 16 + fr;
        if (ml >= rows_m) continue;
        const float sa = p.sa_row ? p.scale_a[m0 + ml] : sa0;
        const float brow = (has_bias && p.transposed) ? load_as_float(p.bias, m0 + ml, p.bias_dtype) : 0.0f;
        uint8_t *row = (uint8_t *)p.C + ((m0 + ml) * p.ldc + n0) * kEsz;
#pragma unroll
        for (int tn = 0; tn < C::TN; ++tn) {
            const int nl = wn0 + tn * 16 + fg * 4;
            if (nl >= cols_n) continue;
            float v[4];
#pragma unroll
            for (int j = 0; j < 4; ++j) {
                float r = p.transposed ? (acc[tn][tm][j] * sbv[tn][j]) * sa : (acc[tn][tm][j] * sa) * sbv[tn][j];
                if (has_bias) r = r + (p.transposed ? brow : bv[tn][j]);
                if (has_sr) r = r * sr;
                v[j] = r;
            }
            uint8_t *dst = row + nl * kEsz;
            if (vec_store && nl + 3 < cols_n) {
                if (OUT == FP8MI_F32) {
                    *(f32x4 *)dst = f32x4{v[0], v[1], v[2], v[3]};
                } else if (OUT == FP8MI_BF16) {
                    __bf16 h0 = (__bf16)v[0], h1 = (__bf16)v[1], h2 = (__bf16)v[2], h3 = (__bf16)v[3];
                    *(u32x2 *)dst = u32x2{(uint32_t)__builtin_bit_cast(uint16_t, h0) | ((uint32_t)__builtin_bit_cast(uint16_t, h1) << 16),
                                          (uint32_t)__builtin_bit_cast(uint16_t, h2) | ((uint32_t)__builtin_bit_cast(uint16_t, h3) << 16)};
                } else {
                    _Float16 h0 = (_Float16)v[0], h1 = (_Float16)v[1], h2 = (_Float16)v[2], h3 = (_Float16)v[3];
                    *(u32x2 *)dst = u32x2{(uint32_t)__builtin_bit_cast(uint16_t, h0) | ((uint32_t)__builtin_bit_cast(uint16_t, h1) << 16),
                                          (uint32_t)__builtin_bit_cast(uint16_t, h2) | ((uint32_t)__builtin_bit_cast(uint16_t, h3) << 16)};
                }
            } else {
#pragma unroll
                for (int j = 0; j < 4; ++j) {
                    if (nl + j < cols_n) {
                        if (OUT == FP8MI_F32) ((float *)dst)[j] = v[j];
                        else if (OUT == FP8MI_BF16) ((__bf16 *)dst)[j] = (__bf16)v[j];
                        else ((_Float16 *)dst)[j] = (_Float16)v[j];
                    }
                }
            }
        }
    }
}

template <typename C, int OUT>
FP8MI_DEVICE void epilogue_staged(const MMParams &p, const EpiScalars &es, const f32x4 (&acc)[C::TN][C::TM], uint8_t *smem, int64_t m0,
                                  int64_t n0, int wave, int wm0, int wn0, int lane)
{
    constexpr int kEsz = OUT == FP8MI_F32 ? 4 : 2;
    constexpr int WNc = C::TN * 16;
    constexpr int kRowBytes = WNc * kEsz;
    constexpr int kStride = kRowBytes + 16;
    constexpr int kCPR = kRowBytes / 16;
    constexpr int kRPI = 64 / kCPR;
    constexpr int kNI = 16 / kRPI;
    static_assert(C::kWaves * 16 * kStride <= C::kRingBytes, "staging fits in the ring");
    uint8_t *buf = smem + wave * (16 * kStride);
    const int fr = lane & 15, fg = lane >> 4;

    const bool has_bias = p.bias != nullptr, has_sr = p.scale_result != nullptr;
    const float sr = es.sr;
    float sbv[C::TN][4], bv[C::TN][4];
    const float sb0 = es.sb0, sa0 = es.sa0;
#pragma unroll
    for (int tn = 0; tn < C::TN; ++tn)
#pragma unroll
        for (int j = 0; j < 4; ++j) {
            const int64_t n = n0 + wn0 + tn * 16 + fg * 4 + j;
            sbv[tn][j] = p.sb_row ? p.scale_b[n] : sb0;
            bv[tn][j] = (has_bias && !p.transposed) ? load_as_float(p.bias, n, p.bias_dtype) : 0.0f;
        }
    const int rrow = lane / kCPR, rchunk = lane % kCPR;
#pragma unroll
    for (int tm = 0; tm < C::TM; ++tm) {
        const float sa = p.sa_row ? p.scale_a[m0 + wm0 + tm * 16 + fr] : sa0;
        const float brow = (has_bias && p.transposed) ? load_as_float(p.bias, m0 + wm0 + tm * 16 + fr, p.bias_dtype) : 0.0f;
#pragma unroll
        for (int tn = 0; tn < C::TN; ++tn) {
            float v[4];
#pragma unroll
            for (int j = 0; j < 4; ++j) {
                float r = p.transposed ? (acc[tn][tm][j] * sbv[tn][j]) * sa : (acc[tn][tm][j] * sa) * sbv[tn][j];
                if (has_bias) r = r + (p.transposed ? brow : bv[tn][j]);
                if (has_sr) r = r * sr;
                v[j] = r;
            }
            uint8_t *d = buf + fr * kStride + (tn * 16 + fg * 4) * kEsz;
            if (OUT == FP8MI_F32) {
                *(f32x4 *)d = f32x4{v[0], v[1], v[2], v[3]};
            } else if (OUT == FP8MI_BF16) {
                __bf16 h0 = (__bf16)v[0], h1 = (__bf16)v[1], h2 = (__bf16)v[2], h3 = (__bf16)v[3];
                *(u32x2 *)d = u32x2{(uint32_t)__builtin_bit_cast(uint16_t, h0) | ((uint32_t)__builtin_bit_cast(uint16_t, h1) << 16),
                                    (uint32_t)__builtin_bit_cast(uint16_t, h2) | ((uint32_t)__builtin_bit_cast(uint16_t, h3) << 16)};
            } else {
                _Float16 h0 = (_Float16)v[0], h1 = (_Float16)v[1], h2 = (_Float16)v[2], h3 = (_Float16)v[3];
                *(u32x2 *)d = u32x2{(uint32_t)__builtin_bit_cast(uint16_t, h0) | ((uint32_t)__builtin_bit_cast(uint16_t, h1) << 16),
                                    (uint32_t)__builtin_bit_cast(uint16_t, h2) | ((uint32_t)__builtin_bit_cast(uint16_t, h3) << 16)};
            }
        }
        uint8_t *grow = (uint8_t *)p.C + ((m0 + wm0 + tm * 16) * p.ldc + n0 + wn0) * kEsz;
#pragma unroll
        for (int i = 0; i < kNI; ++i) {
            const int r = i * kRPI + rrow;
            u32x4 q = *(const u32x4 *)(buf + r * kStride + rchunk * 16);
            store_c16(q, grow + (int64_t)r * p.ldc * kEsz + rchunk * 16);
        }
    }
}

constexpr int kFlagBytes = 16;

template <typename C>
FP8MI_DEVICE bool acc_has_nan(const f32x4 (&acc)[C::TN][C::TM])
{
    f32x4 t = acc[0][0];
#pragma unroll
    for (int tn = 0; tn < C::TN; ++tn)
#pragma unroll
        for (int tm = 0; tm < C::TM; ++tm)
            if (tn + tm) t += acc[tn][tm];
    const float s = (t[0] + t[1]) + (t[2] + t[3]);
    return s != s;
}

FP8MI_DEVICE void tile_of_block(int bid, int nwg, int tiles_m, int tiles_n, int &tile_m, int &tile_n, int &kslice, int &wg)
{
    const int q = nwg >> 3, r = nwg & 7, xcd = bid & 7;
    const int wg_all = (xcd < r ? xcd * (q + 1) : r * (q + 1) + (xcd - r) * q) + (bid >> 3);
    const int n_tiles = tiles_m * tiles_n;
    kslice = wg_all < n_tiles ? 0 : wg_all / n_tiles;
    wg = wg_all - kslice * n_tiles;
    constexpr int kGroupM = 4;
    const int per_group = kGroupM * tiles_n;
    const int group = wg < per_group ? 0 : wg / per_group, first_m = group * kGroupM;
    const int gm = min(kGroupM, tiles_m - first_m);
    const int in_group = wg - group * per_group;
    if (gm == kGroupM) {
        tile_m = first_m + (in_group & (kGroupM - 1));
        tile_n = in_group >> 2;
    } else {
        tile_m = first_m + in_group % gm;
        tile_n = in_group / gm;
    }
}

template <typename C, typename = void> struct xlocal_of { static constexpr bool value = false; };
template <typename C> struct xlocal_of<C, std::void_t<decltype(C::XLOCAL)>> { static constexpr bool value = C::XLOCAL; };

template <typename C>
FP8MI_DEVICE bool splitk_combine(const MMParams &p, f32x4 (&acc)[C::TN][C::TM], uint8_t *smem, int wg, int kslice, int nsplit,
                                 int n_tiles)
{
    constexpr bool kXLocal = xlocal_of<C>::value;
    constexpr int kCoherent = kXLocal ? 1 : 17;
    int *counters = (int *)p.ws;
    constexpr int kVecPerWg = C::TN * C::TM * C::kCThreads;
    __amdgpu_buffer_rsrc_t rw = __builtin_amdgcn_make_buffer_rsrc(
        (void *)(p.ws + kWsCounterBytes), 0, (int)min(p.ws_bytes - kWsCounterBytes, (int64_t)0x7FFFFFFF), 0x00020000);
    const uint32_t slice_bytes = (uint32_t)n_tiles * kVecPerWg * 16u;
    const uint32_t my_off = ((uint32_t)wg * kVecPerWg + threadIdx.x) * 16u;
#pragma unroll
    for (int tn = 0; tn < C::TN; ++tn)
#pragma unroll
        for (int tm = 0; tm < C::TM; ++tm)
            __builtin_amdgcn_raw_buffer_store_b128(__builtin_bit_cast(u32x4, acc[tn][tm]), rw,
                                                   (int)(my_off + (tn * C::TM + tm) * C::kCThreads * 16u),
                                                   (int)((uint32_t)kslice * slice_bytes), kCoherent);
    asm volatile("s_waitcnt vmcnt(0)" ::: "memory");
    volatile int *flag = (volatile int *)smem;
    __syncthreads();
    if (threadIdx.x == 0) *flag = kXLocal ? __hip_atomic_fetch_add(&counters[wg], 1, __ATOMIC_RELAXED, __HIP_MEMORY_SCOPE_WORKGROUP)
                                            : __hip_atomic_fetch_add(&counters[wg], 1, __ATOMIC_RELAXED, __HIP_MEMORY_SCOPE_SYSTEM);
    __syncthreads();
    const int arrived = *flag;
    if (arrived != nsplit - 1) return false;
    constexpr int kQuads = C::TN * C::TM;
    constexpr int kBatch = kQuads <= 4 ? 4 : (kQuads <= 8 ? 3 : (kQuads <= 16 ? 2 : 1));
    for (int s0 = 0; s0 < nsplit; s0 += kBatch) {
        f32x4 v[kBatch][C::TN][C::TM];
#pragma unroll
        for (int b = 0; b < kBatch; ++b) {
            const int s2 = min(s0 + b, nsplit - 1);
#pragma unroll
            for (int tn = 0; tn < C::TN; ++tn)
#pragma unroll
                for (int tm = 0; tm < C::TM; ++tm)
                    v[b][tn][tm] = __builtin_bit_cast(f32x4, __builtin_amdgcn_raw_buffer_load_b128(
                        rw, (int)(my_off + (tn * C::TM + tm) * C::kCThreads * 16u), (int)((uint32_t)s2 * slice_bytes), kCoherent));
        }
#pragma unroll
        for (int b = 0; b < kBatch; ++b) {
            if (s0 + b < nsplit) {
#pragma unroll
                for (int tn = 0; tn < C::TN; ++tn)
#pragma unroll
                    for (int tm = 0; tm < C::TM; ++tm) acc[tn][tm] = (s0 + b == 0) ? v[b][tn][tm] : acc[tn][tm] + v[b][tn][tm];
            }
        }
    }
    if (threadIdx.x == 0) {
        if (kXLocal) __hip_atomic_store(&counters[wg], 0, __ATOMIC_RELAXED, __HIP_MEMORY_SCOPE_WORKGROUP);
        else __hip_atomic_store(&counters[wg], 0, __ATOMIC_RELAXED, __HIP_MEMORY_SCOPE_SYSTEM);
    }
    __syncthreads();
    return true;
}

inline int resolve_split(MMParams &p, int64_t tm, int64_t tn, int BM, int BN, int stage_k)
{
    const int64_t ns_all = (p.K + stage_k - 1) / stage_k;
    const int64_t cus = fp8mi_cu_count();
    int64_t split = p.split > 1 ? p.split : 1;
    if (p.split == 0 && tm * tn <= cus / 2 && ns_all >= 8) {
        split = cus / (tm * tn);
        if (split > ns_all / 4) split = ns_all / 4;
        if (split > 16) split = 16;
    }
    if (!p.ws || tm * tn > kWsCounterBytes / 4) split = 1;
    if (split > ns_all) split = ns_all > 0 ? ns_all : 1;
    if (split > 1) {
        const int64_t per_slice = tm * tn * (int64_t)BM * BN * 4;
        int64_t fit = (p.ws_bytes - kWsCounterBytes) / per_slice;
        if ((int64_t)0x7FFFFFFF / per_slice < fit) fit = (int64_t)0x7FFFFFFF / per_slice;
        if (split > fit) split = fit > 1 ? fit : 1;
    }
    if (split > 1) {
        const int64_t per = (ns_all + split - 1) / split;
        split = (ns_all + per - 1) / per;
        if (tm * tn * split > 0x7FFFFFFF) return FP8MI_E_UNSUPPORTED;
    }
    p.split = (int)split;
    return 0;
}

}
```

### fp8-mps-metal_amd/csrc/fp8mi_gemv.hip

```cpp

#include "fp8mi_common.h"

namespace {


template <bool E5M2 = false>
FP8MI_DEVICE void decode16(const u32x4 &w, f32x2 (&f)[8])
{
#pragma unroll
    for (int j = 0; j < 4; ++j) {
        if constexpr (E5M2) {
            f[2 * j] = __builtin_amdgcn_cvt_pk_f32_bf8(w[j], false);
            f[2 * j + 1] = __builtin_amdgcn_cvt_pk_f32_bf8(w[j], true);
        } else {
            f[2 * j] = __builtin_amdgcn_cvt_pk_f32_fp8(w[j], false);
            f[2 * j + 1] = __builtin_amdgcn_cvt_pk_f32_fp8(w[j], true);
        }
    }
}

template <int STEPS, int RB, bool NT = true, int kWaves = 4, int ABL = 0, bool MFMA = false, int OCC = 0, int FMT = 0>
__global__ __launch_bounds__(kWaves * 64) void gemv_kernel(MMParams p_in)
{
    if constexpr (OCC > 0) {
        __shared__ int occ_pad[(160 * 1024 / OCC - 512) / 4];
        if (p_in.debug == 0x7FFFFFFF) occ_pad[threadIdx.x] = 1;
    }
    const MMParams p = pin_params(p_in);
    const float sr = p.scale_result ? p.scale_result[0] : 1.0f;
    const float sx = p.scale_a[0];
    const float sw0 = p.scale_b[0];
    constexpr int kThreads = kWaves * 64;
    __shared__ float part[kWaves][RB];
    __shared__ int dirty_rows[RB];

    const int lane = threadIdx.x & 63;
    const int wave = threadIdx.x >> 6;
    const int64_t row0 = (int64_t)blockIdx.x * RB;
    const int64_t K = p.K;
    const uint8_t *__restrict__ x = p.A;
    const uint8_t *__restrict__ W = p.B;

    f32x2 acc[RB];
    [[maybe_unused]] f32x4 macc[RB];
#pragma unroll
    for (int r = 0; r < RB; ++r) {
        acc[r] = f32x2{0.0f, 0.0f};
        if constexpr (MFMA) macc[r] = f32x4{0.0f, 0.0f, 0.0f, 0.0f};
    }

    constexpr int64_t kChunk = (int64_t)kWaves * STEPS * 1024;
    for (int64_t kc = 0; kc < K; kc += kChunk) {
        int64_t kb[STEPS];
        bool kv[STEPS];
#pragma unroll
        for (int i = 0; i < STEPS; ++i) {
            kb[i] = kc + (int64_t)(wave + kWaves * i) * 1024 + lane * 16;
            kv[i] = kb[i] < K;
        }
        u32x4 xr[STEPS];
#pragma unroll
        for (int i = 0; i < STEPS; ++i) {
            xr[i] = u32x4{0u, 0u, 0u, 0u};
            if (kv[i]) xr[i] = *(const u32x4 *)(x + kb[i]);
        }
        u32x4 w[RB][STEPS];
#pragma unroll
        for (int r = 0; r < RB; ++r) {
            const bool rv = row0 + r < p.N;
            const uint8_t *wr = W + (row0 + r) * p.ldb;
#pragma unroll
            for (int i = 0; i < STEPS; ++i) {
                if (rv && kv[i]) w[r][i] = NT ? __builtin_nontemporal_load((const u32x4 *)(wr + kb[i])) : *(const u32x4 *)(wr + kb[i]);
                else w[r][i] = u32x4{0u, 0u, 0u, 0u};
            }
        }
        if (FMT == 0 && p.nan_zero) {
#pragma unroll
            for (int i = 0; i < STEPS; ++i)
#pragma unroll
                for (int j = 0; j < 4; ++j) xr[i][j] = scrub_nan4(xr[i][j]);
        }
        if constexpr (MFMA) {
#pragma unroll
            for (int r = 0; r < RB; ++r) {
#pragma unroll
                for (int i = 0; i < STEPS; i += 2) {
                    const u32x4 w1 = i + 1 < STEPS ? w[r][i + 1] : u32x4{0u, 0u, 0u, 0u};
                    const u32x4 x1 = i + 1 < STEPS ? xr[i + 1] : u32x4{0u, 0u, 0u, 0u};
                    const i32x8 a = {(int)w[r][i][0], (int)w[r][i][1], (int)w[r][i][2], (int)w[r][i][3], (int)w1[0], (int)w1[1], (int)w1[2], (int)w1[3]};
                    const i32x8 b = {(int)xr[i][0], (int)xr[i][1], (int)xr[i][2], (int)xr[i][3], (int)x1[0], (int)x1[1], (int)x1[2], (int)x1[3]};
                    macc[r] = __builtin_amdgcn_mfma_scale_f32_16x16x128_f8f6f4(a, b, macc[r], (FMT >> 1) & 1, FMT & 1, 0, 0x7F7F7F7F, 0, 0x7F7F7F7F);
                }
            }
        } else {
            f32x2 xs[STEPS][8];
#pragma unroll
            for (int i = 0; i < STEPS; ++i) decode16<(FMT & 1) != 0>(xr[i], xs[i]);
#pragma unroll
            for (int r = 0; r < RB; ++r) {
#pragma unroll
                for (int i = 0; i < STEPS; ++i) {
                    if constexpr (ABL == 1) {
                        acc[r][0] += __uint_as_float((w[r][i][0] ^ w[r][i][1] ^ w[r][i][2] ^ w[r][i][3]) & 0x3FFFFFFFu);
                        continue;
                    }
                    f32x2 wf[8];
                    decode16<(FMT & 2) != 0>(w[r][i], wf);
#pragma unroll
                    for (int j = 0; j < 8; ++j) acc[r] = xs[i][j] * wf[j] + acc[r];
                }
            }
        }
    }

    if constexpr (MFMA) {
        const int fr = lane & 15, fg = lane >> 4;
        const bool on_diag = (fr >> 2) == fg;
#pragma unroll
        for (int r = 0; r < RB; ++r) {
            const float d = (fr & 2) ? ((fr & 1) ? macc[r][3] : macc[r][2]) : ((fr & 1) ? macc[r][1] : macc[r][0]);
            acc[r] = f32x2{on_diag ? d : 0.0f, 0.0f};
        }
    }

#pragma unroll
    for (int r = 0; r < RB; ++r) {
        float s = wave_sum(acc[r][0] + acc[r][1]);
        if (lane == 0) part[wave][r] = s;
    }
    __syncthreads();

    int dirty = 0;
    if (threadIdx.x < RB) {
        const int r = threadIdx.x;
        const int64_t n = row0 + r;
        float sum = 0.0f;
#pragma unroll
        for (int wv = 0; wv < kWaves; ++wv) sum += part[wv][r];
        dirty = (FMT == 0 && p.nan_zero && sum != sum) ? 1 : 0;
        dirty_rows[r] = dirty;
        if (n < p.N && !dirty) {
            const float sw = p.sb_row ? p.scale_b[n] : sw0;
            const float b = p.bias ? load_as_float(p.bias, p.transposed ? 0 : n, p.bias_dtype) : 0.0f;
            store_from_float(p.C, n, epilogue_value(sum, sx, sw, p.bias != nullptr, b, p.scale_result != nullptr, sr, p.transposed != 0),
                             p.out_dtype);
        }
    }
    if constexpr (FMT != 0) return;
    if (!__syncthreads_or(dirty)) return;

    for (int r = 0; r < RB; ++r) {
        if (!dirty_rows[r]) continue;
        const int64_t n = row0 + r;
        const uint8_t *wr = W + n * p.ldb;
        float s = 0.0f;
        for (int64_t k = threadIdx.x; k < K; k += kThreads) s += decode_ref(x[k]) * decode_ref(wr[k]);
        s = wave_sum(s);
        __syncthreads();
        if (lane == 0) part[wave][0] = s;
        __syncthreads();
        if (threadIdx.x == 0) {
            float sum = 0.0f;
#pragma unroll
            for (int wv = 0; wv < kWaves; ++wv) sum += part[wv][0];
            const float sw = p.sb_row ? p.scale_b[n] : sw0;
            const float b = p.bias ? load_as_float(p.bias, p.transposed ? 0 : n, p.bias_dtype) : 0.0f;
            store_from_float(p.C, n, epilogue_value(sum, sx, sw, p.bias != nullptr, b, p.scale_result != nullptr, sr, p.transposed != 0),
                             p.out_dtype);
        }
    }
}

template <int STEPS, int RB, int MX, int G, int kWaves = 4, bool SWEEP = false, int FMT = 0>
__global__ __launch_bounds__(kWaves * 64) void gemv_mx_kernel(MMParams p_in)
{
    constexpr int kRows = RB * G;
    const MMParams p = pin_params(p_in);
    const float sr = p.scale_result ? p.scale_result[0] : 1.0f;
    const float sa0 = p.scale_a[0];
    const float sw0 = p.scale_b[0];
    constexpr int kThreads = kWaves * 64;
    __shared__ float part[kWaves][MX][kRows][16];
    __shared__ float dump[kWaves][64];
    __shared__ int dirty_cell[MX][kRows];

    const int lane = threadIdx.x & 63;
    const int wave = threadIdx.x >> 6;
    const int64_t row0 = (int64_t)blockIdx.x * kRows;
    auto rown = [&](int r) -> int64_t {
        return SWEEP ? ((int64_t)(r / RB) * gridDim.x + blockIdx.x) * RB + (r % RB) : row0 + r;
    };
    const int64_t K = p.K;
    const uint8_t *__restrict__ X = p.A;
    const uint8_t *__restrict__ W = p.B;
    const int M = (int)p.M;
    const int fr = lane & 15, fg = lane >> 4;
    const bool on_diag = (fr >> 2) == fg;

    f32x4 macc[MX][RB];
    {
        const int64_t kc = 0;
        int64_t kb[STEPS];
        bool kv[STEPS];
#pragma unroll
        for (int i = 0; i < STEPS; ++i) {
            kb[i] = kc + (int64_t)(wave + kWaves * i) * 1024 + lane * 16;
            kv[i] = kb[i] < K;
        }
        u32x4 xr[MX][STEPS];
#pragma unroll
        for (int m = 0; m < MX; ++m)
#pragma unroll
            for (int i = 0; i < STEPS; ++i) {
                xr[m][i] = u32x4{0u, 0u, 0u, 0u};
                if (m < M && kv[i]) xr[m][i] = *(const u32x4 *)(X + (int64_t)m * p.lda + kb[i]);
            }
        auto load_group = [&](int g, u32x4 (&w)[RB][STEPS]) {
#pragma unroll
            for (int r = 0; r < RB; ++r) {
                const int64_t n = rown(g * RB + r);
                const uint8_t *wr = W + n * p.ldb;
#pragma unroll
                for (int i = 0; i < STEPS; ++i) {
                    if (n < p.N && kv[i]) w[r][i] = __builtin_nontemporal_load((const u32x4 *)(wr + kb[i]));
                    else w[r][i] = u32x4{0u, 0u, 0u, 0u};
                }
            }
        };
        auto mul_group = [&](int g, const u32x4 (&w)[RB][STEPS]) {
#pragma unroll
            for (int m = 0; m < MX; ++m)
#pragma unroll
                for (int r = 0; r < RB; ++r) macc[m][r] = f32x4{0.0f, 0.0f, 0.0f, 0.0f};
#pragma unroll
            for (int r = 0; r < RB; ++r) {
#pragma unroll
                for (int i = 0; i < STEPS; i += 2) {
                    const u32x4 w1 = i + 1 < STEPS ? w[r][i + 1] : u32x4{0u, 0u, 0u, 0u};
                    const i32x8 a = {(int)w[r][i][0], (int)w[r][i][1], (int)w[r][i][2], (int)w[r][i][3], (int)w1[0], (int)w1[1], (int)w1[2], (int)w1[3]};
#pragma unroll
                    for (int m = 0; m < MX; ++m) {
                        const u32x4 x0 = xr[m][i], x1 = i + 1 < STEPS ? xr[m][i + 1] : u32x4{0u, 0u, 0u, 0u};
                        const i32x8 b = {(int)x0[0], (int)x0[1], (int)x0[2], (int)x0[3], (int)x1[0], (int)x1[1], (int)x1[2], (int)x1[3]};
                        macc[m][r] = __builtin_amdgcn_mfma_scale_f32_16x16x128_f8f6f4(a, b, macc[m][r], (FMT >> 1) & 1, FMT & 1, 0, 0x7F7F7F7F, 0, 0x7F7F7F7F);
                    }
                }
            }
#pragma unroll
            for (int m = 0; m < MX; ++m)
#pragma unroll
                for (int r = 0; r < RB; ++r) {
                    const float d = (fr & 2) ? ((fr & 1) ? macc[m][r][3] : macc[m][r][2]) : ((fr & 1) ? macc[m][r][1] : macc[m][r][0]);
                    float *cell = on_diag ? &part[wave][m][g * RB + r][fr] : &dump[wave][lane];
                    *cell = d;
                }
        };
        u32x4 wa[RB][STEPS], wb[RB][STEPS];
        load_group(0, wa);
        if (FMT == 0 && p.nan_zero) {
#pragma unroll
            for (int m = 0; m < MX; ++m)
#pragma unroll
                for (int i = 0; i < STEPS; ++i)
#pragma unroll
                    for (int j = 0; j < 4; ++j) xr[m][i][j] = scrub_nan4(xr[m][i][j]);
        }
#pragma unroll
        for (int g = 0; g < G; g += 2) {
            if (g + 1 < G) load_group(g + 1, wb);
            mul_group(g, wa);
            if (g + 1 < G) {
                if (g + 2 < G) load_group(g + 2, wa);
                mul_group(g + 1, wb);
            }
        }
    }
    __syncthreads();

    int dirty = 0;
    constexpr int kCells = MX * kRows, kVals = kWaves * 16;
    constexpr int kP = kThreads / kCells >= 16 ? 16 : (kThreads / kCells >= 8 ? 8 : (kThreads / kCells >= 4 ? 4 : (kThreads / kCells >= 2 ? 2 : 1)));
    const int cell = threadIdx.x / kP, cj = threadIdx.x % kP;
    const int cm = cell / kRows, cr = cell % kRows;
    auto finish = [&](int m, int r, float sum) {
        const int64_t n = rown(r);
        const float sa = p.sa_row ? p.scale_a[m] : sa0;
        const float sw = p.sb_row ? p.scale_b[n] : sw0;
        const float b = p.bias ? load_as_float(p.bias, p.transposed ? (int64_t)m : n, p.bias_dtype) : 0.0f;
        store_from_float(p.C, (int64_t)m * p.ldc + n,
                         epilogue_value(sum, sa, sw, p.bias != nullptr, b, p.scale_result != nullptr, sr, p.transposed != 0), p.out_dtype);
    };
    static_assert(MX * kRows <= kThreads, "one thread per output cell of the workgroup");
    if (threadIdx.x < kCells * kP) {
        float sum = 0.0f;
#pragma unroll
        for (int v = 0; v < kVals / kP; ++v) {
            const int i = v * kP + cj;
            sum += part[i >> 4][cm][cr][i & 15];
        }
        sum = group_sum<kP>(sum);
        dirty = (FMT == 0 && p.nan_zero && sum != sum) ? 1 : 0;
        if (cj == 0) {
            dirty_cell[cm][cr] = dirty;
            if (cm < M && rown(cr) < p.N && !dirty) finish(cm, cr, sum);
        }
    }
    if constexpr (FMT != 0) return;
    if (!__syncthreads_or(dirty)) return;

    float *red = &part[0][0][0][0];
    for (int m = 0; m < M; ++m)
        for (int r = 0; r < kRows; ++r) {
            if (!dirty_cell[m][r]) continue;
            const int64_t n = rown(r);
            if (n >= p.N) continue;
            const uint8_t *wr = W + n * p.ldb;
            const uint8_t *xm = X + (int64_t)m * p.lda;
            float sv = 0.0f;
            for (int64_t k = threadIdx.x; k < K; k += kThreads) sv += decode_ref(xm[k]) * decode_ref(wr[k]);
            sv = wave_sum(sv);
            __syncthreads();
            if (lane == 0) red[wave] = sv;
            __syncthreads();
            if (threadIdx.x == 0) {
                float sum = 0.0f;
#pragma unroll
                for (int wv = 0; wv < kWaves; ++wv) sum += red[wv];
                finish(m, r, sum);
            }
        }
}

template <int STEPS, int RB, int MX, int G, int kWaves = 4, bool SWEEP = false, int FMT = 0>
int launch_mx(const MMParams &p, hipStream_t s)
{
    const int64_t grid = (p.N + RB * G - 1) / (RB * G);
    return fp8mi_launch(gemv_mx_kernel<STEPS, RB, MX, G, kWaves, SWEEP, FMT>, dim3((unsigned)grid), dim3(kWaves * 64), s, p);
}

template <int STEPS, int RB, bool NT = true, int kWaves = 4, int ABL = 0, bool MFMA = false, int OCC = 0, int FMT = 0>
int launch(const MMParams &p, hipStream_t s)
{
    const int64_t grid = (p.N + RB - 1) / RB;
    return fp8mi_launch(gemv_kernel<STEPS, RB, NT, kWaves, ABL, MFMA, OCC, FMT>, dim3((unsigned)grid), dim3(kWaves * 64), s, p);
}

}

bool fp8mi_gemv_supported(const MMParams &p)
{
    return p.M == 1 && p.K > 0 && (p.K % 16) == 0 && (p.ldb % 16) == 0 && (((uintptr_t)p.A) & 15u) == 0 &&
           (((uintptr_t)p.B) & 15u) == 0 && (p.N + 3) / 4 <= 0x7FFFFFFF;
}

bool fp8mi_gemv_mx_supported(const MMParams &p)
{
    return p.M >= 2 && p.M <= 8 && p.K > 0 && p.K <= 16384 && (p.K % 16) == 0 && (p.lda % 16) == 0 && (p.ldb % 16) == 0 && (((uintptr_t)p.A) & 15u) == 0 &&
           (((uintptr_t)p.B) & 15u) == 0 && (p.N + 1) / 2 <= 0x7FFFFFFF;
}

int fp8mi_launch_gemv_mx_variant(const MMParams &p, int id, hipStream_t s);

template <int FMT>
static int launch_gemv_mx_fmt(const MMParams &p, hipStream_t s)
{
    const int64_t steps = (p.K + 4095) / 4096;
    if (p.M <= 2) {
        if (steps <= 1) return launch_mx<1, 2, 2, 4, 4, false, FMT>(p, s);
        if (steps <= 2) return launch_mx<2, 2, 2, 4, 4, false, FMT>(p, s);
        return launch_mx<4, 2, 2, 4, 4, false, FMT>(p, s);
    }
    if (p.M <= 4) {
        if (steps <= 1) return launch_mx<1, 2, 4, 4, 4, false, FMT>(p, s);
        if (steps <= 2) return launch_mx<2, 2, 4, 4, 4, false, FMT>(p, s);
        return launch_mx<4, 2, 4, 4, 4, false, FMT>(p, s);
    }
    if (steps <= 1) return launch_mx<1, 2, 8, 4, 4, false, FMT>(p, s);
    if (steps <= 2) return launch_mx<2, 2, 8, 8, 4, false, FMT>(p, s);
    return launch_mx<2, 2, 8, 8, 8, false, FMT>(p, s);
}

int fp8mi_launch_gemv_mx(const MMParams &p, hipStream_t s, int fmt)
{
    switch (fmt) {
    case 0: return launch_gemv_mx_fmt<0>(p, s);
    case 1: return launch_gemv_mx_fmt<1>(p, s);
    case 2: return launch_gemv_mx_fmt<2>(p, s);
    case 3: return launch_gemv_mx_fmt<3>(p, s);
    default: return FP8MI_E_ENUM;
    }
}

#ifdef FP8MI_DIAG
int fp8mi_launch_gemv_mx_variant(const MMParams &p, int id, hipStream_t s)
{
    const int64_t steps = (p.K + 4095) / 4096;
    const bool sweep = id >= 74;
    const int v = sweep ? id - 74 : id - 70;
    const int g = v == 0 ? 1 : (v == 1 ? 2 : (v == 2 ? 4 : 8));
#define MXV(S, MXN)                                                             \
    (sweep ? (g == 1 ? launch_mx<S, 2, MXN, 1, 4, true>(p, s) : g == 2 ? launch_mx<S, 2, MXN, 2, 4, true>(p, s) \
              : g == 4 ? launch_mx<S, 2, MXN, 4, 4, true>(p, s) : launch_mx<S, 2, MXN, 8, 4, true>(p, s))        \
           : (g == 1 ? launch_mx<S, 2, MXN, 1>(p, s) : g == 2 ? launch_mx<S, 2, MXN, 2>(p, s) \
              : g == 4 ? launch_mx<S, 2, MXN, 4>(p, s) : launch_mx<S, 2, MXN, 8>(p, s)))
    if (p.M <= 2) return steps <= 1 ? MXV(1, 2) : steps <= 2 ? MXV(2, 2) : MXV(4, 2);
    if (p.M <= 4) return steps <= 1 ? MXV(1, 4) : steps <= 2 ? MXV(2, 4) : MXV(4, 4);
    if (steps <= 2) return steps <= 1 ? MXV(1, 8) : MXV(2, 8);
    return g == 1 ? launch_mx<2, 2, 8, 1, 8>(p, s) : g == 2 ? launch_mx<2, 2, 8, 2, 8>(p, s) : g == 4 ? launch_mx<2, 2, 8, 4, 8>(p, s) : launch_mx<2, 2, 8, 8, 8>(p, s);
#undef MXV
}
#endif

#ifdef FP8MI_DIAG
int fp8mi_launch_gemv_variant(const MMParams &p, int id, hipStream_t s)
{
    switch (id) {
    case 40: return launch<4, 8>(p, s);
    case 41: return launch<4, 4>(p, s);
    case 42: return launch<2, 8, true, 8>(p, s);
    case 43: return launch<2, 4, true, 8>(p, s);
    case 44: return launch<4, 8, false>(p, s);
    case 45: return launch<2, 2, true, 8>(p, s);
    case 46: return launch<4, 2>(p, s);
    case 47: return launch<1, 8, true, 16>(p, s);
    case 48: return launch<2, 4, true, 8, 1>(p, s);
    case 49: return launch<4, 8, true, 4, 1>(p, s);
    case 50: return launch<4, 8, true, 4, 0, true>(p, s);
    case 51: return launch<2, 4, true, 8, 0, true>(p, s);
    case 52: return launch<4, 4, true, 4, 0, true>(p, s);
    case 53: return launch<2, 8, true, 8, 0, true>(p, s);
    case 54: return launch<4, 2, true, 4, 0, true>(p, s);
    case 55: return launch<2, 2, true, 8, 0, true>(p, s);
    case 56: return launch<2, 4, true, 4, 0, true>(p, s);
    case 57: return launch<2, 8, true, 4, 0, true>(p, s);
    case 58: return launch<1, 4, true, 4, 0, true>(p, s);
    case 59: return launch<1, 2, true, 4, 0, true>(p, s);
    case 60: return launch<1, 8, true, 4, 0, true>(p, s);
    case 61: return launch<1, 2>(p, s);
    case 180: return launch<1, 1>(p, s);
    case 181: return launch<1, 8>(p, s);
    case 182: return launch<1, 2, true, 4, 0, false, 4>(p, s);
    case 183: return launch<1, 4, false>(p, s);
    case 62: return launch<2, 2, true, 4, 0, true>(p, s);
    case 63: return launch<4, 1, true, 4, 0, true>(p, s);
    case 64: return launch<1, 1, true, 4, 0, true>(p, s);
    case 65: return launch<4, 2, true, 4, 0, true, 2>(p, s);
    case 66: return launch<4, 2, true, 4, 0, true, 3>(p, s);
    case 67: return launch<4, 2, true, 4, 0, true, 4>(p, s);
    case 68: return launch<4, 2, true, 4, 0, true, 6>(p, s);
    case 69: return launch<4, 1, true, 4, 0, true, 4>(p, s);
    case 160: return launch<4, 1, true, 4, 0, true, 6>(p, s);
    case 161: return launch<4, 4, true, 4, 0, true, 2>(p, s);
    case 162: return launch_mx<4, 2, 1, 2>(p, s);
    case 163: return launch_mx<4, 2, 1, 4>(p, s);
    case 164: return launch_mx<4, 2, 1, 8>(p, s);
    case 165: return launch_mx<4, 1, 1, 8>(p, s);
    case 166: return launch_mx<4, 1, 1, 4>(p, s);
    case 167: return launch_mx<4, 1, 1, 16>(p, s);
    case 168: return launch_mx<2, 1, 1, 8>(p, s);
    case 169: return launch_mx<2, 2, 1, 4>(p, s);
    case 170: return launch_mx<2, 1, 1, 8, 8>(p, s);
    case 171: return launch_mx<2, 2, 1, 4, 8>(p, s);
    case 174: return launch_mx<4, 1, 1, 4, 4, true>(p, s);
    case 175: return launch_mx<4, 1, 1, 8, 4, true>(p, s);
    case 176: return launch_mx<4, 2, 1, 4, 4, true>(p, s);
    case 177: return launch_mx<4, 2, 1, 2, 4, true>(p, s);
    case 178: return launch_mx<4, 1, 1, 16, 4, true>(p, s);
    case 179: return launch_mx<2, 2, 1, 4, 4, true>(p, s);
    case 172: return launch_mx<1, 2, 1, 4>(p, s);
    case 173: return launch_mx<1, 1, 1, 8>(p, s);
    default: return FP8MI_E_ENUM;
    }
}
#endif

template <int FMT>
static int launch_gemv_fmt(const MMParams &p, bool fp32_only, hipStream_t s)
{
    const int64_t steps = (p.K + 4095) / 4096;
    if (steps <= 1) return launch<1, 4, true, 4, 0, false, 0, FMT>(p, s);
    if (fp32_only) {
        if (steps <= 2) return launch<2, 4, true, 4, 0, false, 0, FMT>(p, s);
        if (p.K > 16384) return launch<2, 4, true, 8, 0, false, 0, FMT>(p, s);
        return launch<4, 2, true, 4, 0, false, 0, FMT>(p, s);
    }
    if (steps <= 2) return launch<2, 2, true, 4, 0, true, 0, FMT>(p, s);
    if (p.K <= 16384 && p.N <= 8192 && p.lda % 16 == 0) return launch_mx<4, 2, 1, 4, 4, true, FMT>(p, s);
    return launch<4, 2, true, 4, 0, true, 0, FMT>(p, s);
}

int fp8mi_launch_gemv(const MMParams &p, bool fp32_only, hipStream_t s, int fmt)
{
    switch (fmt) {
    case 0: return launch_gemv_fmt<0>(p, fp32_only, s);
    case 1: return launch_gemv_fmt<1>(p, fp32_only, s);
    case 2: return launch_gemv_fmt<2>(p, fp32_only, s);
    case 3: return launch_gemv_fmt<3>(p, fp32_only, s);
    default: return FP8MI_E_ENUM;
    }
}
```

Baseline: 1097 TFLOP/s.

## Issue GEMM prologue loads before scalar setup and use constant-space scale loads

Moves the initial pipeline-stage global loads out of run_tile into an earlier issue_prologue call in the kernel body, so the first tile loads go out before the epilogue scale loads, the LDS flag init and the scale-plan setup. The scale reads now go through the constant address space (address_space 4), so they can be scalar loads, and the LDS flag accesses use explicit address_space(3) pointers instead of generic volatile pointers. The intent is to shorten kernel startup latency before the first MFMA. A STAGED template flag keeps the old in-function prologue for the NaN-scrub rerun path, which adds complexity.

```diff
diff --git a/fp8-mps-metal_amd/csrc/diag/fp8mi_gemm_pc.hip b/fp8-mps-metal_amd/csrc/diag/fp8mi_gemm_pc.hip
--- a/fp8-mps-metal_amd/csrc/diag/fp8mi_gemm_pc.hip
+++ b/fp8-mps-metal_amd/csrc/diag/fp8mi_gemm_pc.hip
@@ -236,7 +236,7 @@
 {
     using C = PCfg<BM, BN, CWM, CWN, NL, NSTAGE, KS, ABL>;
     __shared__ __attribute__((aligned(16))) uint8_t smem[C::kRingBytes + kFlagBytes];
-    if (threadIdx.x == 0) *(volatile int *)(smem + C::kRingBytes) = 0;
+    if (threadIdx.x == 0) *lds_word(smem + C::kRingBytes) = 0;
     const MMParams p = pin_params(p_in);
     FP8MI_PIN_S(tiles_m); FP8MI_PIN_S(tiles_n); FP8MI_PIN_S(vec_store); FP8MI_PIN_S(nwg);
     const EpiScalars es = load_epi_scalars(p);
@@ -258,7 +258,7 @@
     const int s0 = kslice * ns_slice, ns = min(ns_slice, ns_all - s0);
     lds_u8 *ring = (lds_u8 *)smem;
 
-    volatile int *flag = (volatile int *)(smem + C::kRingBytes);
+    lds_vint *flag = lds_word(smem + C::kRingBytes);
 
     if (is_loader) {
         const int64_t bytes_a = (rows_a - 1) * p.lda + p.K, bytes_b = (rows_b - 1) * p.ldb + p.K;
diff --git a/fp8-mps-metal_amd/csrc/fp8mi_common.h b/fp8-mps-metal_amd/csrc/fp8mi_common.h
--- a/fp8-mps-metal_amd/csrc/fp8mi_common.h
+++ b/fp8-mps-metal_amd/csrc/fp8mi_common.h
@@ -87,6 +87,8 @@
     FP8MI_PIN_S(q.transposed); FP8MI_PIN_S(q.nan_zero); FP8MI_PIN_S(q.split); FP8MI_PIN_S(q.ws); FP8MI_PIN_S(q.ws_bytes);
     return q;
 }
+
+FP8MI_DEVICE float load_uniform_f32(const float *p) { return *(const __attribute__((address_space(4))) float *)p; }
 
 #ifndef FP8MI_CSTORE
 #define FP8MI_CSTORE 1
diff --git a/fp8-mps-metal_amd/csrc/fp8mi_gemm.hip b/fp8-mps-metal_amd/csrc/fp8mi_gemm.hip
--- a/fp8-mps-metal_amd/csrc/fp8mi_gemm.hip
+++ b/fp8-mps-metal_amd/csrc/fp8mi_gemm.hip
@@ -353,12 +353,27 @@
     else issue_stage<C, false>(pl, ra, rb, stage, wave, step * (BK * C::KS), K);
 }
 
+template <typename C>
+FP8MI_DEVICE void issue_prologue(const StagePlan<C> &pl, __amdgpu_buffer_rsrc_t ra, __amdgpu_buffer_rsrc_t rb, uint8_t *smem, int wave,
+                                 int ks0, int nk, int rot, int64_t K)
+{
+    const int nk_all = (int)((K + BK * C::KS - 1) / (BK * C::KS));
+    const bool ktail = (K % (BK * C::KS)) != 0;
+    int ks = rot;
+#pragma unroll
+    for (int s = 0; s < C::PF; ++s)
+        if (s < nk) {
+            issue_any<C>(pl, ra, rb, smem + s * C::kStageBytes, wave, ks0 + ks, nk_all, ktail, K);
+            ks = (ks + 1 == nk) ? 0 : ks + 1;
+        }
+}
+
 FP8MI_DEVICE void prefetch_stage(uint32_t &sink, uint32_t voff, u32x4 rsrc, uint32_t koff)
 {
     asm volatile("buffer_load_dword %0, %1, %2, %3 offen" : "+v"(sink) : "v"(voff), "s"(rsrc), "s"(koff) : "memory");
 }
 
-template <typename C, bool SCRUB>
+template <typename C, bool SCRUB, bool STAGED>
 FP8MI_DEVICE void run_tile(const MMParams &p, uint8_t *smem, const StagePlan<C> &pl, __amdgpu_buffer_rsrc_t ra,
                            __amdgpu_buffer_rsrc_t rb, int wave, int wm0, int wn0, uint32_t off1, uint32_t off2,
                            int ks0, int nk, int rot, const MxLane<C> &ml, f32x4 (&acc)[C::TN][C::TM])
@@ -384,7 +399,10 @@
 
 #pragma unroll
     for (int s = 0; s < C::PF; ++s)
-        if (s < nk) issue_any<C>(pl, ra, rb, smem + s * C::kStageBytes, wave, next_ks(), nk_all, ktail, K);
+        if (s < nk) {
+            const int first = next_ks();
+            if constexpr (!STAGED) issue_any<C>(pl, ra, rb, smem + s * C::kStageBytes, wave, first, nk_all, ktail, K);
+        }
 #pragma unroll
     for (int s = 0; s < C::PFD; ++s) prefetch(C::PF + s);
 
@@ -467,12 +485,14 @@
     STAMP(p2_);
     if ((threadIdx.x & 63) == 0 && blockIdx.x < 256 && wave == 0) {
         unsigned long long *o = g_stamp + blockIdx.x * 32 + 26;
-        o[0] = p0_; o[1] = p1_; o[2] = p2_;
-    }
-#endif
-}
-
-template <typename C, bool SCRUB>
+        if (!STAGED) o[0] = p0_;
+        o[1] = p1_; o[2] = p2_;
+    }
+    if (!STAGED && (threadIdx.x & 63) == 0 && blockIdx.x < 256 && wave == 1) g_stamp[blockIdx.x * 32 + 14] = p0_;
+#endif
+}
+
+template <typename C, bool SCRUB, bool STAGED>
 FP8MI_DEVICE void run_tile_staggered(const MMParams &p, uint8_t *smem, const StagePlan<C> &pl, __amdgpu_buffer_rsrc_t ra,
                                      __amdgpu_buffer_rsrc_t rb, int wave, int wm0, int wn0, uint32_t off1, uint32_t off2,
                                      int ks0, int nk, int rot, const MxLane<C> &ml, f32x4 (&acc)[C::TN][C::TM])
@@ -491,7 +511,10 @@
     auto next_ks = [&]() { const int r = ks; ks = (ks + 1 == nk) ? 0 : ks + 1; return ks0 + r; };
 #pragma unroll
     for (int s = 0; s < C::PF; ++s)
-        if (s < nk) issue_any<C>(pl, ra, rb, smem + s * C::kStageBytes, wave, next_ks(), nk_all, ktail, K);
+        if (s < nk) {
+            const int first = next_ks();
+            if constexpr (!STAGED) issue_any<C>(pl, ra, rb, smem + s * C::kStageBytes, wave, first, nk_all, ktail, K);
+        }
     int slot = 0, fill = C::PF % C::NSTAGE;
     auto advance = [&]() {
         slot = (slot + 1 == C::NSTAGE) ? 0 : slot + 1;
@@ -544,13 +567,13 @@
 #undef FP8MI_MULTIPLY
 }
 
-template <typename C, bool SCRUB>
+template <typename C, bool SCRUB, bool STAGED>
 FP8MI_DEVICE void run_tile_any(const MMParams &p, uint8_t *smem, const StagePlan<C> &pl, __amdgpu_buffer_rsrc_t ra,
                                __amdgpu_buffer_rsrc_t rb, int wave, int wm0, int wn0, uint32_t off1, uint32_t off2,
                                int ks0, int nk, int rot, const MxLane<C> &ml, f32x4 (&acc)[C::TN][C::TM])
 {
-    if constexpr (C::MODE == 2) run_tile_staggered<C, SCRUB>(p, smem, pl, ra, rb, wave, wm0, wn0, off1, off2, ks0, nk, rot, ml, acc);
-    else run_tile<C, SCRUB>(p, smem, pl, ra, rb, wave, wm0, wn0, off1, off2, ks0, nk, rot, ml, acc);
+    if constexpr (C::MODE == 2) run_tile_staggered<C, SCRUB, STAGED>(p, smem, pl, ra, rb, wave, wm0, wn0, off1, off2, ks0, nk, rot, ml, acc);
+    else run_tile<C, SCRUB, STAGED>(p, smem, pl, ra, rb, wave, wm0, wn0, off1, off2, ks0, nk, rot, ml, acc);
 }
 
 using MxArgs = MxScales;
@@ -560,13 +583,11 @@
 };
 
 template <typename C, typename S>
-FP8MI_DEVICE void gemm_tile(const MMParams &p, const S &mx, const EpiScalars &es, uint8_t *smem, int tiles_m, int tiles_n,
-                            int vec_store, int nwg)
+FP8MI_DEVICE void gemm_tile(const MMParams &p, const S &mx, uint8_t *smem, int tiles_m, int tiles_n, int vec_store, int nwg)
 {
     constexpr int BM = C::kWavesM * (C::TM * 16), BN = C::kWavesN * (C::TN * 16), WM = C::TM * 16, WN = C::TN * 16;
-    if (!C::FP4 && !C::OCP && threadIdx.x == 0) *(volatile int *)(smem + C::kRingBytes) = 0;
-
-    unsigned long long k0_ = 0, k1_ = 0, k2_ = 0; (void)k0_; (void)k1_; (void)k2_;
+
+    unsigned long long k0_ = 0, k1_ = 0, k2_ = 0, d0_ = 0; (void)k0_; (void)k1_; (void)k2_; (void)d0_;
     STAMP(k0_);
 #ifdef FP8MI_STAMP
     const unsigned long long r0_ = __builtin_amdgcn_s_memrealtime();
@@ -622,6 +643,56 @@
             for (int o = (int)threadIdx.x * 16; o < C::kRingBytes; o += C::kThreads * 16) *(u32x4 *)(smem + o) = u32x4{0u, 0u, 0u, 0u};
             __syncthreads();
         }
+    }
+    if constexpr (C::BW) {
+        const int64_t bx0 = m0 >> mx.sh_a, bw0 = n0 >> mx.sh_b;
+        const int64_t nbx = ((m0 + rows_a - 1) >> mx.sh_a) - bx0 + 1, nbw = ((n0 + rows_b - 1) >> mx.sh_b) - bw0 + 1;
+        const int64_t ext_x = ((nbx - 1) * mx.sa_sr + (mx.nkb - 1) * mx.sa_sk + 1) * 4, ext_w = ((nbw - 1) * mx.sb_sr + (mx.nkb - 1) * mx.sb_sk + 1) * 4;
+        pl.sc.rx = __builtin_amdgcn_make_buffer_rsrc((void *)(mx.sa + bx0 * mx.sa_sr), 0, (int)min(ext_x, (int64_t)0x7FFFFFFF), 0x00020000);
+        pl.sc.rw = __builtin_amdgcn_make_buffer_rsrc((void *)(mx.sb + bw0 * mx.sb_sr), 0, (int)min(ext_w, (int64_t)0x7FFFFFFF), 0x00020000);
+        pl.sc.kx = (uint32_t)(mx.sa_sk * 4);
+        pl.sc.kw = (uint32_t)(mx.sb_sk * 4);
+        pl.sc.nkb = (int)mx.nkb;
+#pragma unroll
+        for (int j = 0; j < C::kScaleLoadsPerWave; ++j) {
+            const int idx = wave + j * C::kLoaders, q = idx / C::kScalePieces, part = idx - q * C::kScalePieces;
+            const bool is_x = part < C::kScalePiecesA;
+            const int row = (is_x ? part : part - C::kScalePiecesA) * 64 + lane;
+            const bool ok = idx < C::KS * C::kScalePieces && row < (is_x ? rows_a : rows_b);
+            const int64_t rb = is_x ? ((m0 + row) >> mx.sh_a) - bx0 : ((n0 + row) >> mx.sh_b) - bw0;
+            pl.sc.voff[j] = ok ? (uint32_t)(rb * (is_x ? mx.sa_sr : mx.sb_sr) * 4 + q * (is_x ? pl.sc.kx : pl.sc.kw)) : kOOB;
+            pl.sc.is_x[j] = is_x;
+            pl.sc.q[j] = q;
+        }
+    } else if constexpr (C::MXS) {
+        pl.sc.rx = __builtin_amdgcn_make_buffer_rsrc((void *)(mx.sx + m0 * mx.ld_sx), 0, (int)min(rows_a * mx.ld_sx, (int64_t)0x7FFFFFFF), 0x00020000);
+        pl.sc.rw = __builtin_amdgcn_make_buffer_rsrc((void *)(mx.sw + n0 * mx.ld_sw), 0, (int)min(rows_b * mx.ld_sw, (int64_t)0x7FFFFFFF), 0x00020000);
+#pragma unroll
+        for (int j = 0; j < C::kScaleLoadsPerWave; ++j) {
+            const int idx = wave + j * C::kLoaders, q = idx / C::kScalePieces, part = idx - q * C::kScalePieces;
+            const bool is_x = part < C::kScalePiecesA;
+            const int row = (is_x ? part : part - C::kScalePiecesA) * 64 + lane;
+            const bool ok = idx < C::KS * C::kScaleHalves * C::kScalePieces && row < (is_x ? rows_a : rows_b);
+            pl.sc.voff[j] = ok ? (uint32_t)(row * (is_x ? mx.ld_sx : mx.ld_sw) + q * 4) : kOOB;
+            pl.sc.is_x[j] = is_x;
+        }
+    }
+    const int nk_all = (int)((p.K + BK * C::KS - 1) / (BK * C::KS));
+    const int nsplit = p.split > 1 ? p.split : 1;
+    const int nk_slice = (nk_all + nsplit - 1) / nsplit;
+    const int ks0 = kslice * nk_slice, nk = min(nk_slice, nk_all - ks0);
+    const int rot = 0;
+
+    STAMP(d0_);
+    if constexpr (C::FLOOR != 2) issue_prologue<C>(pl, ra, rb, smem, wave, ks0, nk, rot, p.K);
+    __builtin_amdgcn_sched_barrier(0);
+#ifdef FP8MI_STAMP
+    if (lane == 0 && blockIdx.x < 256 && wave <= 1) g_stamp[blockIdx.x * 32 + (wave ? 14 : 26)] = d0_;
+#endif
+
+    const EpiScalars es = load_epi_scalars<C::MXS>(p);
+    if (!C::FP4 && !C::OCP && threadIdx.x == 0) *lds_word(smem + C::kRingBytes) = 0;
+    {
         if (C::PFD > 0) {
             constexpr int kLines = BN * C::KS / 4;
             static_assert(C::PFD == 0 || kLines <= 64, "one prefetch instruction per stage");
@@ -653,41 +724,11 @@
 
     MxLane<C> ml;
     if constexpr (C::BW) {
-        const int64_t bx0 = m0 >> mx.sh_a, bw0 = n0 >> mx.sh_b;
-        const int64_t nbx = ((m0 + rows_a - 1) >> mx.sh_a) - bx0 + 1, nbw = ((n0 + rows_b - 1) >> mx.sh_b) - bw0 + 1;
-        const int64_t ext_x = ((nbx - 1) * mx.sa_sr + (mx.nkb - 1) * mx.sa_sk + 1) * 4, ext_w = ((nbw - 1) * mx.sb_sr + (mx.nkb - 1) * mx.sb_sk + 1) * 4;
-        pl.sc.rx = __builtin_amdgcn_make_buffer_rsrc((void *)(mx.sa + bx0 * mx.sa_sr), 0, (int)min(ext_x, (int64_t)0x7FFFFFFF), 0x00020000);
-        pl.sc.rw = __builtin_amdgcn_make_buffer_rsrc((void *)(mx.sb + bw0 * mx.sb_sr), 0, (int)min(ext_w, (int64_t)0x7FFFFFFF), 0x00020000);
-        pl.sc.kx = (uint32_t)(mx.sa_sk * 4);
-        pl.sc.kw = (uint32_t)(mx.sb_sk * 4);
-        pl.sc.nkb = (int)mx.nkb;
-#pragma unroll
-        for (int j = 0; j < C::kScaleLoadsPerWave; ++j) {
-            const int idx = wave + j * C::kLoaders, q = idx / C::kScalePieces, part = idx - q * C::kScalePieces;
-            const bool is_x = part < C::kScalePiecesA;
-            const int row = (is_x ? part : part - C::kScalePiecesA) * 64 + lane;
-            const bool ok = idx < C::KS * C::kScalePieces && row < (is_x ? rows_a : rows_b);
-            const int64_t rb = is_x ? ((m0 + row) >> mx.sh_a) - bx0 : ((n0 + row) >> mx.sh_b) - bw0;
-            pl.sc.voff[j] = ok ? (uint32_t)(rb * (is_x ? mx.sa_sr : mx.sb_sr) * 4 + q * (is_x ? pl.sc.kx : pl.sc.kw)) : kOOB;
-            pl.sc.is_x[j] = is_x;
-            pl.sc.q[j] = q;
-        }
         ml.xo = (uint32_t)((wm0 + fr) * 4);
         ml.wo = (uint32_t)(C::kScalePiecesA * 256 + (wn0 + fg * 4) * 4);
         ml.rows_ok = 0;
         ml.kend = 0;
     } else if constexpr (C::MXS) {
-        pl.sc.rx = __builtin_amdgcn_make_buffer_rsrc((void *)(mx.sx + m0 * mx.ld_sx), 0, (int)min(rows_a * mx.ld_sx, (int64_t)0x7FFFFFFF), 0x00020000);
-        pl.sc.rw = __builtin_amdgcn_make_buffer_rsrc((void *)(mx.sw + n0 * mx.ld_sw), 0, (int)min(rows_b * mx.ld_sw, (int64_t)0x7FFFFFFF), 0x00020000);
-#pragma unroll
-        for (int j = 0; j < C::kScaleLoadsPerWave; ++j) {
-            const int idx = wave + j * C::kLoaders, q = idx / C::kScalePieces, part = idx - q * C::kScalePieces;
-            const bool is_x = part < C::kScalePiecesA;
-            const int row = (is_x ? part : part - C::kScalePiecesA) * 64 + lane;
-            const bool ok = idx < C::KS * C::kScaleHalves * C::kScalePieces && row < (is_x ? rows_a : rows_b);
-            pl.sc.voff[j] = ok ? (uint32_t)(row * (is_x ? mx.ld_sx : mx.ld_sw) + q * 4) : kOOB;
-            pl.sc.is_x[j] = is_x;
-        }
         ml.xo = (uint32_t)((wm0 + fr) * 4 + fg);
         ml.wo = (uint32_t)(C::kScalePiecesA * 256 + (wn0 + fr) * 4 + fg);
         uint32_t ok = 0;
@@ -699,12 +740,6 @@
         ml.kend = p.K - (C::FP4 ? 16 : 32) * fg;
     }
 
-    const int nk_all = (int)((p.K + BK * C::KS - 1) / (BK * C::KS));
-    const int nsplit = p.split > 1 ? p.split : 1;
-    const int nk_slice = (nk_all + nsplit - 1) / nsplit;
-    const int ks0 = kslice * nk_slice, nk = min(nk_slice, nk_all - ks0);
-    const int rot = 0;
-
     f32x4 acc[C::TN][C::TM];
     if constexpr (C::FLOOR == 2) {
 #pragma unroll
@@ -712,18 +747,18 @@
 #pragma unroll
             for (int tm = 0; tm < C::TM; ++tm) acc[tn][tm] = f32x4{0.0f, 0.0f, 0.0f, 0.0f};
     } else
-    run_tile_any<C, false>(p, smem, pl, ra, rb, wave, wm0, wn0, off1, off2, ks0, nk, rot, ml, acc);
+    run_tile_any<C, false, true>(p, smem, pl, ra, rb, wave, wm0, wn0, off1, off2, ks0, nk, rot, ml, acc);
 
     if constexpr (C::FP4 || C::OCP) {
         asm volatile("s_waitcnt lgkmcnt(0)" ::: "memory");
         __builtin_amdgcn_s_barrier();
     } else {
-        volatile int *flag = (volatile int *)(smem + C::kRingBytes);
+        lds_vint *flag = lds_word(smem + C::kRingBytes);
         if (p.nan_zero && acc_has_nan<C>(acc)) *flag = 1;
         asm volatile("s_waitcnt lgkmcnt(0)" ::: "memory");
         __builtin_amdgcn_s_barrier();
         if (p.nan_zero && *flag) {
-            run_tile_any<C, true>(p, smem, pl, ra, rb, wave, wm0, wn0, off1, off2, ks0, nk, rot, ml, acc);
+            run_tile_any<C, true, false>(p, smem, pl, ra, rb, wave, wm0, wn0, off1, off2, ks0, nk, rot, ml, acc);
             asm volatile("s_waitcnt lgkmcnt(0)" ::: "memory");
             __builtin_amdgcn_s_barrier();
         }
@@ -764,17 +799,17 @@
 __global__ __launch_bounds__((Cfg<BM, BN, WM, WN, NSTAGE, PP, ABL, KS, LD>::kThreads)) void gemm_kernel(MMParams p_in, int tiles_m, int tiles_n, int vec_store, int nwg)
 {
     using C = Cfg<BM, BN, WM, WN, NSTAGE, PP, ABL, KS, LD>;
+    unsigned long long e0_ = 0; (void)e0_;
+    STAMP(e0_);
     const MMParams p = pin_params(p_in);
     FP8MI_PIN_S(tiles_m); FP8MI_PIN_S(tiles_n); FP8MI_PIN_S(vec_store); FP8MI_PIN_S(nwg);
     if constexpr (C::FLOOR == 3) {
         if (p.M < 0) *(volatile int *)p.C = tiles_m + tiles_n + vec_store + nwg;
         return;
     }
-    const EpiScalars es = load_epi_scalars(p);
     __shared__ __attribute__((aligned(16))) uint8_t smem[C::kRingBytes + kFlagBytes];
-    if (threadIdx.x == 0) *(volatile int *)(smem + C::kRingBytes) = 0;
-
-    unsigned long long k0_ = 0, k1_ = 0, k2_ = 0; (void)k0_; (void)k1_; (void)k2_;
+
+    unsigned long long k0_ = 0, k1_ = 0, k2_ = 0, d0_ = 0; (void)k0_; (void)k1_; (void)k2_; (void)d0_;
     STAMP(k0_);
 #ifdef FP8MI_STAMP
     const unsigned long long r0_ = __builtin_amdgcn_s_memrealtime();
@@ -797,6 +832,9 @@
     const int wave = __builtin_amdgcn_readfirstlane(threadIdx.x >> 6);
     const int wm0 = (wave % C::kWavesM) * WM;
     const int wn0 = (wave / C::kWavesM) * WN;
+#ifdef FP8MI_STAMP
+    if (lane == 0 && blockIdx.x < 256 && wave <= 1) g_stamp[blockIdx.x * 32 + (wave ? 13 : 31)] = e0_;
+#endif
 
     const int64_t rows_a = min((int64_t)BM, p.M - m0), rows_b = min((int64_t)BN, p.N - n0);
     const int64_t bytes_a = (rows_a - 1) * p.lda + p.K, bytes_b = (rows_b - 1) * p.ldb + p.K;
@@ -830,6 +868,23 @@
             for (int o = (int)threadIdx.x * 16; o < C::kRingBytes; o += C::kThreads * 16) *(u32x4 *)(smem + o) = u32x4{0u, 0u, 0u, 0u};
             __syncthreads();
         }
+    }
+    const int nk_all = (int)((p.K + BK * C::KS - 1) / (BK * C::KS));
+    const int nsplit = p.split > 1 ? p.split : 1;
+    const int nk_slice = (nk_all + nsplit - 1) / nsplit;
+    const int ks0 = kslice * nk_slice, nk = min(nk_slice, nk_all - ks0);
+    const int rot = 0;
+
+    STAMP(d0_);
+    if constexpr (C::FLOOR != 2) issue_prologue<C>(pl, ra, rb, smem, wave, ks0, nk, rot, p.K);
+    __builtin_amdgcn_sched_barrier(0);
+#ifdef FP8MI_STAMP
+    if (lane == 0 && blockIdx.x < 256 && wave <= 1) g_stamp[blockIdx.x * 32 + (wave ? 14 : 26)] = d0_;
+#endif
+
+    const EpiScalars es = load_epi_scalars(p);
+    if (threadIdx.x == 0) *lds_word(smem + C::kRingBytes) = 0;
+    {
         if (C::PFD > 0) {
             constexpr int kLines = BN * C::KS / 4;
             static_assert(C::PFD == 0 || kLines <= 64, "one prefetch instruction per stage");
@@ -859,12 +914,6 @@
     const uint32_t off1 = (uint32_t)(fr * BK + ((fg ^ (fr >> 1)) << 4));
     const uint32_t off2 = (uint32_t)(fr * BK + (((4 + fg) ^ (fr >> 1)) << 4));
 
-    const int nk_all = (int)((p.K + BK * C::KS - 1) / (BK * C::KS));
-    const int nsplit = p.split > 1 ? p.split : 1;
-    const int nk_slice = (nk_all + nsplit - 1) / nsplit;
-    const int ks0 = kslice * nk_slice, nk = min(nk_slice, nk_all - ks0);
-    const int rot = 0;
-
     f32x4 acc[C::TN][C::TM];
     if constexpr (C::FLOOR == 2) {
 #pragma unroll
@@ -872,14 +921,14 @@
 #pragma unroll
             for (int tm = 0; tm < C::TM; ++tm) acc[tn][tm] = f32x4{0.0f, 0.0f, 0.0f, 0.0f};
     } else
-    run_tile_any<C, false>(p, smem, pl, ra, rb, wave, wm0, wn0, off1, off2, ks0, nk, rot, MxLane<C>{}, acc);
-
-    volatile int *flag = (volatile int *)(smem + C::kRingBytes);
+    run_tile_any<C, false, true>(p, smem, pl, ra, rb, wave, wm0, wn0, off1, off2, ks0, nk, rot, MxLane<C>{}, acc);
+
+    lds_vint *flag = lds_word(smem + C::kRingBytes);
     if (p.nan_zero && acc_has_nan<C>(acc)) *flag = 1;
     asm volatile("s_waitcnt lgkmcnt(0)" ::: "memory");
     __builtin_amdgcn_s_barrier();
     if (p.nan_zero && *flag) {
-        run_tile_any<C, true>(p, smem, pl, ra, rb, wave, wm0, wn0, off1, off2, ks0, nk, rot, MxLane<C>{}, acc);
+        run_tile_any<C, true, false>(p, smem, pl, ra, rb, wave, wm0, wn0, off1, off2, ks0, nk, rot, MxLane<C>{}, acc);
         asm volatile("s_waitcnt lgkmcnt(0)" ::: "memory");
         __builtin_amdgcn_s_barrier();
     }
@@ -924,12 +973,8 @@
     MxArgs mx = px.s;
     FP8MI_PIN_S(mx.sx); FP8MI_PIN_S(mx.sw); FP8MI_PIN_S(mx.ld_sx); FP8MI_PIN_S(mx.ld_sw);
     FP8MI_PIN_S(tiles_m); FP8MI_PIN_S(tiles_n); FP8MI_PIN_S(vec_store); FP8MI_PIN_S(nwg);
-    EpiScalars es;
-    es.sa0 = 1.0f;
-    es.sb0 = 1.0f;
-    es.sr = p.scale_result ? p.scale_result[0] : 1.0f;
     __shared__ __attribute__((aligned(16))) uint8_t smem[C::kRingBytes + kFlagBytes];
-    gemm_tile<C>(p, mx, es, smem, tiles_m, tiles_n, vec_store, nwg);
+    gemm_tile<C>(p, mx, smem, tiles_m, tiles_n, vec_store, nwg);
 }
 
 template <int BM, int BN, int WM, int WN, int NSTAGE, int PP, int ABL, int KS, int LD>
@@ -941,12 +986,8 @@
     MxArgs mx = px.s;
     FP8MI_PIN_S(mx.sx); FP8MI_PIN_S(mx.sw); FP8MI_PIN_S(mx.ld_sx); FP8MI_PIN_S(mx.ld_sw);
     FP8MI_PIN_S(tiles_m); FP8MI_PIN_S(tiles_n); FP8MI_PIN_S(vec_store); FP8MI_PIN_S(nwg);
-    EpiScalars es;
-    es.sa0 = 1.0f;
-    es.sb0 = 1.0f;
-    es.sr = p.scale_result ? p.scale_result[0] : 1.0f;
     __shared__ __attribute__((aligned(16))) uint8_t smem[C::kRingBytes + kFlagBytes];
-    gemm_tile<C>(p, mx, es, smem, tiles_m, tiles_n, vec_store, nwg);
+    gemm_tile<C>(p, mx, smem, tiles_m, tiles_n, vec_store, nwg);
 }
 
 struct BwParams {
@@ -965,12 +1006,8 @@
     FP8MI_PIN_S(bs.sa); FP8MI_PIN_S(bs.sb); FP8MI_PIN_S(bs.sa_sr); FP8MI_PIN_S(bs.sa_sk); FP8MI_PIN_S(bs.sb_sr); FP8MI_PIN_S(bs.sb_sk);
     FP8MI_PIN_S(bs.nkb); FP8MI_PIN_S(bs.sh_a); FP8MI_PIN_S(bs.sh_b);
     FP8MI_PIN_S(tiles_m); FP8MI_PIN_S(tiles_n); FP8MI_PIN_S(vec_store); FP8MI_PIN_S(nwg);
-    EpiScalars es;
-    es.sa0 = 1.0f;
-    es.sb0 = 1.0f;
-    es.sr = p.scale_result ? p.scale_result[0] : 1.0f;
     __shared__ __attribute__((aligned(16))) uint8_t smem[C::kRingBytes + kFlagBytes];
-    gemm_tile<C>(p, bs, es, smem, tiles_m, tiles_n, vec_store, nwg);
+    gemm_tile<C>(p, bs, smem, tiles_m, tiles_n, vec_store, nwg);
 }
 
 #ifndef FP8MI_FLOOR_PROBE
@@ -983,9 +1020,8 @@
     static_assert(C::OCP && C::FLOOR == 0 && !C::BREG && !C::XLOCAL, "the e5m2 forms are built from product configurations only");
     const MMParams p = pin_params(p_in);
     FP8MI_PIN_S(tiles_m); FP8MI_PIN_S(tiles_n); FP8MI_PIN_S(vec_store); FP8MI_PIN_S(nwg);
-    const EpiScalars es = load_epi_scalars(p);
     __shared__ __attribute__((aligned(16))) uint8_t smem[C::kRingBytes + kFlagBytes];
-    gemm_tile<C>(p, NoScales{}, es, smem, tiles_m, tiles_n, vec_store, nwg);
+    gemm_tile<C>(p, NoScales{}, smem, tiles_m, tiles_n, vec_store, nwg);
 }
 
 #endif
diff --git a/fp8-mps-metal_amd/csrc/fp8mi_gemm_epi.h b/fp8-mps-metal_amd/csrc/fp8mi_gemm_epi.h
--- a/fp8-mps-metal_amd/csrc/fp8mi_gemm_epi.h
+++ b/fp8-mps-metal_amd/csrc/fp8mi_gemm_epi.h
@@ -10,17 +10,20 @@
 static_assert(kWsCounterBytes == FP8MI_WS_COUNTER_BYTES, "include/fp8mi.h and the kernels agree on the counter block");
 
 typedef __attribute__((address_space(3))) void lds_void;
+typedef __attribute__((address_space(3))) volatile int lds_vint;
+FP8MI_DEVICE lds_vint *lds_word(uint8_t *smem_byte) { return (lds_vint *)(lds_void *)smem_byte; }
 
 struct EpiScalars {
     float sa0, sb0, sr;
 };
 
+template <bool UNIT = false>
 FP8MI_DEVICE EpiScalars load_epi_scalars(const MMParams &p)
 {
     EpiScalars e;
-    e.sa0 = p.scale_a[0];
-    e.sb0 = p.scale_b[0];
-    e.sr = p.scale_result ? p.scale_result[0] : 1.0f;
+    e.sa0 = UNIT ? 1.0f : load_uniform_f32(p.scale_a);
+    e.sb0 = UNIT ? 1.0f : load_uniform_f32(p.scale_b);
+    e.sr = p.scale_result ? load_uniform_f32(p.scale_result) : 1.0f;
     return e;
 }
 
@@ -213,7 +216,7 @@
                                                    (int)(my_off + (tn * C::TM + tm) * C::kCThreads * 16u),
                                                    (int)((uint32_t)kslice * slice_bytes), kCoherent);
     asm volatile("s_waitcnt vmcnt(0)" ::: "memory");
-    volatile int *flag = (volatile int *)smem;
+    lds_vint *flag = lds_word(smem);
     __syncthreads();
     if (threadIdx.x == 0) *flag = kXLocal ? __hip_atomic_fetch_add(&counters[wg], 1, __ATOMIC_RELAXED, __HIP_MEMORY_SCOPE_WORKGROUP)
                                             : __hip_atomic_fetch_add(&counters[wg], 1, __ATOMIC_RELAXED, __HIP_MEMORY_SCOPE_SYSTEM);
diff --git a/fp8-mps-metal_amd/csrc/fp8mi_gemv.hip b/fp8-mps-metal_amd/csrc/fp8mi_gemv.hip
--- a/fp8-mps-metal_amd/csrc/fp8mi_gemv.hip
+++ b/fp8-mps-metal_amd/csrc/fp8mi_gemv.hip
@@ -27,9 +27,9 @@
         if (p_in.debug == 0x7FFFFFFF) occ_pad[threadIdx.x] = 1;
     }
     const MMParams p = pin_params(p_in);
-    const float sr = p.scale_result ? p.scale_result[0] : 1.0f;
-    const float sx = p.scale_a[0];
-    const float sw0 = p.scale_b[0];
+    const float sr = p.scale_result ? load_uniform_f32(p.scale_result) : 1.0f;
+    const float sx = load_uniform_f32(p.scale_a);
+    const float sw0 = load_uniform_f32(p.scale_b);
     constexpr int kThreads = kWaves * 64;
     __shared__ float part[kWaves][RB];
     __shared__ int dirty_rows[RB];
@@ -177,9 +177,9 @@
 {
     constexpr int kRows = RB * G;
     const MMParams p = pin_params(p_in);
-    const float sr = p.scale_result ? p.scale_result[0] : 1.0f;
-    const float sa0 = p.scale_a[0];
-    const float sw0 = p.scale_b[0];
+    const float sr = p.scale_result ? load_uniform_f32(p.scale_result) : 1.0f;
+    const float sa0 = load_uniform_f32(p.scale_a);
+    const float sw0 = load_uniform_f32(p.scale_b);
     constexpr int kThreads = kWaves * 64;
     __shared__ float part[kWaves][MX][kRows][16];
     __shared__ float dump[kWaves][64];
```

Measured after the change: 1114 TFLOP/s, median of 6. 1.01x the previous value.
